# LuxGraph/Lux

Measured on NVIDIA H100. Metric: MTEPS, higher is better.
Workload: dtype f32

## Files before the change

lux_b200/csrc/api.cu:

```cuda
#include <cub/cub.cuh>
#include <stdarg.h>
#include <stdlib.h>
#include <string.h>
#include <algorithm>
#include <new>

#include "build.cuh"
#include "cf.cuh"
#include "pull.cuh"
#include "panel.cuh"
#include "seg.cuh"
#include "push.cuh"
#include "runtime.cuh"
#include <thrust/iterator/counting_iterator.h>

using namespace luxb;

enum class AppRun : uint8_t { kIterations, kConvergence, kEntry };
static constexpr char kBcRun[] = "luxb_bc_run";

struct AppInfo {
  const char* name;
  AppRun run;
  const char* entry;
  bool weights;
  bool dist_labels;
  uint32_t vbytes;
  bool check;
  bool settable;
};
static constexpr AppInfo kApps[] = {
    {"pagerank",                        AppRun::kIterations,  nullptr,          false,  false, 4,        false, true},
    {"connected components",            AppRun::kConvergence, nullptr,          false,  false, 4,        true,  true},
    {"SSSP",                            AppRun::kConvergence, nullptr,          false,  false, 4,        true,  true},
    {"col_filter",                      AppRun::kIterations,  nullptr,          true,   false, 4 * kCfK, false, true},
    {"weighted SSSP",                   AppRun::kConvergence, nullptr,          true,   true,  4,        true,  true},
    {"betweenness centrality",          AppRun::kEntry,       kBcRun,           false,  false, 8,        false, true},
    {"weighted betweenness centrality", AppRun::kEntry,       kBcRun,           true,   true,  8,        false, true},
    {"triangle counting",               AppRun::kEntry,       "luxb_tc_run",    false,  false, 8,        false, false},
    {"k-core decomposition",            AppRun::kEntry,       "luxb_kcore_run", false,  false, 4,        true,  true},
    {"k-truss decomposition",           AppRun::kEntry,       "luxb_truss_run", false,  false, 4,        true,  false},
};
static constexpr int kNumApps = sizeof(kApps) / sizeof(kApps[0]);
static_assert(kNumApps == LUXB_TRUSS + 1, "one row per luxb_app");
static const AppInfo& app_of(const luxb_graph* g) { return kApps[g->cfg.app]; }

static const char* const kPhaseName[12] = {"pull_tile", "fixup", "refresh", "rechunk", "barrier", "panel", "combine", "pack+push", "pull/bcast", "cold_hub", "bc_sigma", "bc_delta"};
static void pt_mark(luxb_graph* g, int tag) {
  PhaseTimer& pt = g->pt;
  if (!pt.on) return;
  cudaEvent_t e;
  cudaEventCreate(&e);
  cudaEventRecord(e, g->stream);
  pt.ev.push_back(e);
  pt.tag.push_back(tag);
}
static void pt_print(luxb_graph* g) {
  if (g->pt.on && g->pt.cnt) {
    char line[1024];
    const bool bc = app_of(g).entry == kBcRun;
    int n = snprintf(line, sizeof(line), "[luxb rank %d] phase means over %ld %s:", g->cfg.rank, g->pt.cnt, bc ? "sources" : "iterations");
    double sum = 0;
    for (int k = bc ? 10 : 0; k < (bc ? 12 : 10); ++k) {
      n += snprintf(line + n, sizeof(line) - n, " %s %.3f ms;", kPhaseName[k], g->pt.sum[k] / g->pt.cnt);
      sum += g->pt.sum[k] / g->pt.cnt;
    }
    snprintf(line + n, sizeof(line) - n, " sum %.3f ms\n", sum);
    fputs(line, stderr);
  }
}

static void pt_flush(luxb_graph* g) {
  PhaseTimer& pt = g->pt;
  if (!pt.on || pt.ev.empty()) return;
  cudaStreamSynchronize(g->stream);
  for (size_t i = 1; i < pt.ev.size(); ++i) {
    if (pt.tag[i] < 0) continue;
    float ms = 0;
    cudaEventElapsedTime(&ms, pt.ev[i - 1], pt.ev[i]);
    pt.sum[pt.tag[i]] += ms;
    if (pt.tag[i] == (app_of(g).entry == kBcRun ? 10 : 0)) pt.cnt++;
  }
  for (cudaEvent_t e : pt.ev) cudaEventDestroy(e);
  pt.ev.clear();
  pt.tag.clear();
}


namespace luxb {
static thread_local char g_err[1024] = "";
void set_error(const char* fmt, ...) {
  va_list ap;
  va_start(ap, fmt);
  vsnprintf(g_err, sizeof(g_err), fmt, ap);
  va_end(ap);
}
}

#define LUXB_ARG(cond, ...)             \
  do {                                  \
    if (!(cond)) {                      \
      set_error(__VA_ARGS__);           \
      return LUXB_ERR_ARG;              \
    }                                   \
  } while (0)

#define LUXB_NCCL(expr)                                                                              \
  do {                                                                                               \
    ncclResult_t _r = (expr);                                                                        \
    if (_r != ncclSuccess) {                                                                         \
      set_error("NCCL error %s at %s:%d: %s", #expr, __FILE__, __LINE__, nccl().GetErrorString(_r)); \
      return LUXB_ERR_COMM;                                                                          \
    }                                                                                                \
  } while (0)

#define LUXB_PULL_SHAPES(X) X(0, 7, 8, 2) X(1, 9, 8, 2) X(2, 7, 16, 2)
#define LUXB_DECL_SHAPE(id, ipt, warps, stages) using PullShape##id = PullShape<ipt, warps, stages>;
LUXB_PULL_SHAPES(LUXB_DECL_SHAPE)
#define LUXB_TILE_OF(id, ipt, warps, stages) PullShape##id::kTile,
static const int kPullTileOf[] = {LUXB_PULL_SHAPES(LUXB_TILE_OF)};
static const int kNumPullShapes = sizeof(kPullTileOf) / sizeof(int);
static const int kDefaultPullShape = 0;
static const int kDefaultPullCtas = 3;

static inline int grid_for(uint64_t n, int threads, int cap) {
  uint64_t b = (n + threads - 1) / threads;
  if (b < 1) b = 1;
  if (b > (uint64_t)cap) b = cap;
  return (int)b;
}

template <class T>
static size_t padded_bytes(uint64_t count) { return std::max<uint64_t>(count, 1) * sizeof(T) + 256; }

template <class T>
static int gmalloc(luxb_graph* g, T** p, uint64_t count, MemKind kind = MemKind::kDevice) {
  void* q = nullptr;
  if (kind == MemKind::kDevice) LUXB_CUDA(cudaMalloc(&q, padded_bytes<T>(count)));
  else if (kind == MemKind::kPinned) LUXB_CUDA(cudaMallocHost(&q, padded_bytes<T>(count)));
  else LUXB_CUDA(cudaHostAlloc(&q, padded_bytes<T>(count), cudaHostAllocMapped | cudaHostAllocPortable));
  g->owned.push_back({q, kind});
  *p = reinterpret_cast<T*>(q);
  return 0;
}

static cudaError_t free_owned(const OwnedBuf& b) { return b.kind == MemKind::kDevice ? cudaFree(b.p) : cudaFreeHost(b.p); }

static int gfree(luxb_graph* g, void* p) {
  for (size_t i = 0; i < g->owned.size(); ++i)
    if (g->owned[i].p == p) {
      const OwnedBuf b = g->owned[i];
      g->owned.erase(g->owned.begin() + i);
      LUXB_CUDA(free_owned(b));
      return 0;
    }
  return 0;
}

template <class T>
static int edge_alloc(luxb_graph* g, T** p, uint64_t count) {
  return gmalloc(g, p, count, g->cfg.zero_copy_edges ? MemKind::kMapped : MemKind::kDevice);
}

struct DevTmp {
  std::vector<void*> ptrs;
  ~DevTmp() { for (void* q : ptrs) cudaFree(q); }
  template <class T>
  int alloc(T** out, uint64_t count) {
    void* q = nullptr;
    LUXB_CUDA(cudaMalloc(&q, padded_bytes<T>(count)));
    ptrs.push_back(q);
    *out = reinterpret_cast<T*>(q);
    return 0;
  }
  void release(void* q) {
    for (size_t i = 0; i < ptrs.size(); ++i)
      if (ptrs[i] == q) { cudaFree(q); ptrs.erase(ptrs.begin() + i); return; }
  }
  void keep(luxb_graph* g, void* q) {
    for (size_t i = 0; i < ptrs.size(); ++i)
      if (ptrs[i] == q) { ptrs.erase(ptrs.begin() + i); g->owned.push_back({q, MemKind::kDevice}); return; }
  }
};

template <class F>
static int cub_call(DevTmp& tmp, cudaStream_t stream, F&& f) {
  size_t bytes = 0;
  LUXB_CUDA(f(nullptr, bytes));
  char* d_tmp = nullptr;
  LUXB_TRY(tmp.alloc(&d_tmp, bytes));
  LUXB_CUDA(f(d_tmp, bytes));
  LUXB_CUDA(cudaStreamSynchronize(stream));
  tmp.release(d_tmp);
  return 0;
}

static int alloc_fixup(luxb_graph* g, FixupScratch& f, uint32_t n_tiles) {
  LUXB_TRY(gmalloc(g, (uint32_t**)&f.d_head, (uint64_t)n_tiles + 1));
  LUXB_TRY(gmalloc(g, (uint32_t**)&f.d_tail, (uint64_t)n_tiles + 1));
  f.n_fix_blocks = (n_tiles + kFixBlock - 1) / kFixBlock;
  LUXB_TRY(gmalloc(g, (uint64_t**)&f.d_carry, (uint64_t)n_tiles + 1));
  LUXB_TRY(gmalloc(g, &f.d_carry_flag, (uint64_t)n_tiles + 1));
  LUXB_TRY(gmalloc(g, (uint64_t**)&f.d_block_agg, (uint64_t)f.n_fix_blocks + 1));
  LUXB_TRY(gmalloc(g, &f.d_block_flag, (uint64_t)f.n_fix_blocks + 1));
  return 0;
}

static int host_partition(uint32_t nv, uint64_t ne, const uint64_t* row_end, int P, uint32_t* rl, uint32_t* np,
                          uint64_t* cl) {
  uint64_t cap = (ne + P - 1) / P;
  uint32_t left = 0;
  int count = 0, found_adjust = 0;
  while (left < nv && count < P) {
    uint64_t base = left == 0 ? 0 : row_end[left - 1];
    const uint64_t* first = std::upper_bound(row_end + left, row_end + nv, base + cap);
    uint32_t v = (uint32_t)(first - row_end);
    if (v < nv) {
      rl[count] = left; np[count] = v - left + 1; cl[count] = base; ++count;
      left = v + 1;
    } else {
      if (row_end[nv - 1] - base == 0) --found_adjust;
      rl[count] = left; np[count] = nv - left; cl[count] = base; ++count;
      left = nv;
    }
  }
  int found = count + found_adjust;
  for (int p = count; p < P; ++p) { rl[p] = nv; np[p] = 0; cl[p] = ne; }
  return found;
}

static constexpr uint32_t kBalanceHubIndeg = 64;
static inline uint64_t vertex_cost(uint64_t indeg) { return 8 + (indeg >= kBalanceHubIndeg ? 4 : 7) * indeg; }

static void host_balanced_partition(uint32_t nv, uint64_t ne, const uint64_t* row_end, int P, uint32_t* rl, uint32_t* np, uint64_t* cl) {
  uint64_t total = 0;
  for (uint32_t v = 0; v < nv; ++v) total += vertex_cost(row_end[v] - (v ? row_end[v - 1] : 0));
  uint64_t run = 0;
  uint32_t left = 0;
  int p = 0;
  for (uint32_t v = 0; v < nv && p < P - 1; ++v) {
    run += vertex_cost(row_end[v] - (v ? row_end[v - 1] : 0));
    if (run * P >= total * (uint64_t)(p + 1)) {
      rl[p] = left; np[p] = v - left + 1; cl[p] = left ? row_end[left - 1] : 0;
      left = v + 1;
      ++p;
    }
  }
  rl[p] = left; np[p] = nv - left; cl[p] = left ? row_end[left - 1] : 0;
  for (++p; p < P; ++p) { rl[p] = nv; np[p] = 0; cl[p] = ne; }
}

static bool use_balanced_split(const luxb_config* cfg) {
  return cfg->balanced_split && cfg->nranks > 1 && (cfg->app == LUXB_PAGERANK || cfg->app == LUXB_COLFILTER);
}

static int check_config(const luxb_config* cfg) {
  LUXB_ARG(cfg != nullptr, "config is NULL");
  LUXB_ARG((unsigned)cfg->app < (unsigned)kNumApps, "unknown app %d", (int)cfg->app);
  LUXB_ARG(cfg->nranks >= 1 && cfg->nranks <= LUXB_MAX_PARTS, "nranks %d out of range [1,%d]", cfg->nranks, LUXB_MAX_PARTS);
  LUXB_ARG(cfg->rank >= 0 && cfg->rank < cfg->nranks, "rank %d out of range", cfg->rank);
  return 0;
}

static int graph_begin(const luxb_config* cfg, uint32_t nv, uint64_t ne, luxb_graph** out) {
  LUXB_TRY(check_config(cfg));
  LUXB_ARG(out != nullptr, "out is NULL");
  int ndev = 0;
  cudaError_t e = cudaGetDeviceCount(&ndev);
  if (e != cudaSuccess || ndev == 0) {
    set_error("no CUDA device available (%s): libluxb has no CPU fallback", cudaGetErrorString(e));
    return LUXB_ERR_CUDA;
  }
  LUXB_ARG(cfg->device >= 0 && cfg->device < ndev, "device %d out of range (have %d)", cfg->device, ndev);
  LUXB_CUDA(cudaSetDevice(cfg->device));
  luxb_graph* g = new (std::nothrow) luxb_graph();
  if (!g) { set_error("out of host memory"); return LUXB_ERR_NOMEM; }
  g->cfg = *cfg;
  g->P = cfg->nranks;
  g->nv = nv;
  g->ne = ne;
  g->weighted = app_of(g).weights;
  *out = g;
  LUXB_CUDA(cudaStreamCreateWithFlags(&g->stream, cudaStreamNonBlocking));
  LUXB_CUDA(cudaEventCreate(&g->ev_begin));
  LUXB_CUDA(cudaEventCreate(&g->ev_end));
  LUXB_CUDA(cudaDeviceGetAttribute(&g->num_sms, cudaDevAttrMultiProcessorCount, cfg->device));
  g->pull_ctas = kDefaultPullCtas;
  if (const char* env = getenv("LUXB_PULL_CTAS")) g->pull_ctas = std::max(1, atoi(env));
  if (const char* env = getenv("LUXB_PHASE_TIMING")) { g->pt.on = atoi(env) != 0; g->pt.per_call = atoi(env) == 2; }
  if (const char* env = getenv("LUXB_L2_HINTS")) g->l2_hints = atoi(env);
  if (const char* env = getenv("LUXB_OVERLAP")) g->overlap_exchange = atoi(env) != 0;
  if (const char* env = getenv("LUXB_BARRIER")) { g->flag_barrier = strcmp(env, "nccl") != 0; g->flag_barrier_all = strcmp(env, "flag") == 0; }
  if (const char* env = getenv("LUXB_PUSH")) g->direct_push = strcmp(env, "direct") == 0;
  if (const char* env = getenv("LUXB_BARRIER_TIMEOUT_S")) g->barrier_timeout_ns = (uint64_t)std::max(1, atoi(env)) * 1000000000ull;
  if (const char* env = getenv("LUXB_FUSED_FIXUP")) g->fused_fixup = atoi(env) != 0;
  if (const char* env = getenv("LUXB_PANEL_RESERVE_SMS")) g->panel_reserve_sms = std::max(0, atoi(env));
  return 0;
}

static void set_partition_derived(luxb_graph* g) {
  int r = g->cfg.rank;
  g->row_left = g->rl[r];
  g->n_part = g->np[r];
  g->col_left = g->cl[r];
  uint64_t next = (r + 1 < g->P) ? g->cl[r + 1] : g->ne;
  if (g->np[r] == 0) next = g->col_left;
  g->e_part = next - g->col_left;
// ... 655 lines not shown
  std::vector<unsigned long long> hist(cap + 1);
  LUXB_CUDA(cudaMemcpyAsync(hist.data(), d_hist, (cap + 1) * 8, cudaMemcpyDeviceToHost, g->stream));
  LUXB_CUDA(cudaStreamSynchronize(g->stream));
  uint64_t above = 0;
  uint32_t tau = cap + 1;
  for (uint32_t d = cap; d >= 2; --d) {
    if (above + hist[d] > h_max) break;
    above += hist[d];
    tau = d;
  }
  if (above == 0 || tau > cap) return 0;
  const uint32_t H = (uint32_t)above;
  if (compact_cold && g->P == 1) {
    const int cs_mode = g->sweep.cs;
    uint64_t e_cold_src = 0;
    for (uint32_t d = 1; d < tau; ++d) e_cold_src += (uint64_t)d * hist[d];
    if (cs_mode == 0 || (cs_mode < 0 && (!split_may_run(g) || g->e_part < kSplitMinEdges ||
                                         (double)e_cold_src < kColdSplitMinShare * (double)g->e_part)))
      compact_cold = false;
  }
  uint64_t *d_keys = nullptr, *d_keys2 = nullptr;
  uint32_t *d_ids = nullptr, *d_ids2 = nullptr, *d_map = nullptr;
  unsigned int* d_cursor = nullptr;
  LUXB_TRY(tmp.alloc(&d_keys, H));
  LUXB_TRY(tmp.alloc(&d_keys2, H));
  LUXB_TRY(tmp.alloc(&d_ids, H));
  LUXB_TRY(tmp.alloc(&d_ids2, H));
  LUXB_TRY(gmalloc(g, &g->d_hot_order, H));
  LUXB_TRY(tmp.alloc(&d_cursor, 1 + LUXB_MAX_PARTS));
  LUXB_CUDA(cudaMemsetAsync(d_cursor, 0, 4 * (1 + LUXB_MAX_PARTS), g->stream));
  PartTable pt{};
  pt.P = g->P;
  for (int p = 0; p < g->P; ++p) { pt.rl[p] = g->rl[p]; pt.np[p] = g->np[p]; }
  hot_select_kernel<<<grid, 256, 0, g->stream>>>(g->d_deg, g->nv, tau, pt, d_cursor, d_cursor + 1, d_keys, d_ids, H);
  LUXB_CUDA(cudaGetLastError());
  int vbits = 1;
  while ((1ull << vbits) < (uint64_t)g->nv) ++vbits;
  LUXB_TRY(cub_call(tmp, g->stream, [&](void* t, size_t& b) {
    return cub::DeviceRadixSort::SortPairs(t, b, d_ids, d_ids2, d_keys, d_keys2, (int)H, 0, vbits, g->stream);
  }));
  LUXB_TRY(cub_call(tmp, g->stream, [&](void* t, size_t& b) {
    return cub::DeviceRadixSort::SortPairs(t, b, d_keys2, d_keys, d_ids2, g->d_hot_order, (int)H, 0, 32, g->stream);
  }));
  unsigned int h_cnt[1 + LUXB_MAX_PARTS];
  LUXB_CUDA(cudaMemcpyAsync(h_cnt, d_cursor, sizeof(h_cnt), cudaMemcpyDeviceToHost, g->stream));
  LUXB_CUDA(cudaStreamSynchronize(g->stream));
  g->hot_off[0] = 0;
  for (int p = 0; p < g->P; ++p) g->hot_off[p + 1] = g->hot_off[p] + h_cnt[1 + p];
  LUXB_TRY(tmp.alloc(&d_map, g->nv));
  uint32_t *d_cflag = nullptr, *d_crank = nullptr;
  if (compact_cold) {
    LUXB_TRY(tmp.alloc(&d_cflag, (uint64_t)g->nv + 1));
    LUXB_TRY(tmp.alloc(&d_crank, (uint64_t)g->nv + 1));
    cold_flag_kernel<<<grid, 256, 0, g->stream>>>(g->d_deg, g->nv, tau, d_cflag);
    LUXB_CUDA(cudaMemsetAsync(d_cflag + g->nv, 0, 4, g->stream));
    LUXB_TRY(cub_call(tmp, g->stream, [&](void* t, size_t& b) {
      return cub::DeviceScan::ExclusiveSum(t, b, d_cflag, d_crank, (int)g->nv + 1, g->stream);
    }));
    for (int p = 0; p <= g->P; ++p) {
      const uint32_t at = p < g->P ? std::min(g->rl[p], g->nv) : g->nv;
      LUXB_CUDA(cudaMemcpyAsync(&g->cold_off[p], d_crank + at, 4, cudaMemcpyDeviceToHost, g->stream));
    }
    LUXB_CUDA(cudaStreamSynchronize(g->stream));
    g->cold_n = g->cold_off[g->P];
    gather_map_compact_kernel<<<grid, 256, 0, g->stream>>>(d_map, d_crank, g->nv, H);
  } else {
    gather_map_init_kernel<<<grid, 256, 0, g->stream>>>(d_map, g->nv, H);
  }
  if (compact_cold && g->P == 1) {
    uint32_t* d_zsrc = nullptr;
    LUXB_TRY(gmalloc(g, &d_zsrc, (uint64_t)H + g->cold_n + 1));
    LUXB_CUDA(cudaMemcpyAsync(d_zsrc, g->d_hot_order, (size_t)H * 4, cudaMemcpyDeviceToDevice, g->stream));
    pack_list_cold_kernel<<<grid, 256, 0, g->stream>>>(d_cflag, d_crank, 0, g->nv, 0, d_zsrc + H);
    LUXB_CUDA(cudaGetLastError());
    LUXB_CUDA(cudaStreamSynchronize(g->stream));
    LUXB_TRY(gfree(g, g->d_hot_order));
    g->d_hot_order = d_zsrc;
    g->cold_z = true;
  } else if (compact_cold) {
    uint32_t *d_okeys = nullptr, *d_okeys2 = nullptr, *d_ranks = nullptr;
    LUXB_TRY(tmp.alloc(&d_okeys, H));
    LUXB_TRY(tmp.alloc(&d_okeys2, H));
    LUXB_TRY(tmp.alloc(&d_ranks, H));
    LUXB_TRY(gmalloc(g, &g->d_zperm, H));
    owner_keys_kernel<<<grid, 256, 0, g->stream>>>(g->d_hot_order, H, pt, d_okeys, d_ranks);
    LUXB_CUDA(cudaGetLastError());
    LUXB_TRY(cub_call(tmp, g->stream, [&](void* t, size_t& b) {
      return cub::DeviceRadixSort::SortPairs(t, b, d_okeys, d_okeys2, d_ranks, g->d_zperm, (int)H, 0, 8, g->stream);
    }));
    const int me = g->cfg.rank;
    const uint32_t nh_me = g->hot_off[me + 1] - g->hot_off[me], nc_me = g->cold_off[me + 1] - g->cold_off[me];
    LUXB_TRY(gmalloc(g, &g->d_pack_list, (uint64_t)nh_me + nc_me + 1));
    if (nh_me)
      pack_list_hot_kernel<<<grid_for(nh_me, 256, grid), 256, 0, g->stream>>>(g->d_hot_order, g->d_zperm, g->hot_off[me], nh_me, g->row_left,
                                                                              g->d_pack_list);
    if (g->n_part)
      pack_list_cold_kernel<<<grid, 256, 0, g->stream>>>(d_cflag, d_crank, g->row_left, g->n_part, g->cold_off[me], g->d_pack_list + nh_me);
    LUXB_CUDA(cudaGetLastError());
    g->packed = true;
  }
  gather_map_hot_kernel<<<grid, 256, 0, g->stream>>>(d_map, g->d_hot_order, H);
  LUXB_TRY(edge_alloc(g, &g->d_src_gather, g->e_part + 8));
  LUXB_CUDA(cudaMemsetAsync(g->d_src_gather, 0, (g->e_part + 8) * 4, g->stream));
  remap_src_kernel<<<grid, 256, 0, g->stream>>>(g->d_src, g->e_part, d_map, g->d_src_gather);
  LUXB_CUDA(cudaGetLastError());
  LUXB_CUDA(cudaStreamSynchronize(g->stream));
  g->hot_n = H;
  return 0;
}

static int allgather_slices(luxb_graph* g, void* replica, size_t elem_bytes);
static void resolve_sweep_settings(SweepSettings& s);
static int build_seg_sweep(luxb_graph* g);
static int pagerank_publish(luxb_graph* g, float* x_new);
static int wait_cold_exchange(luxb_graph* g);
static int bc_alloc(luxb_graph* g);
static int tc_build(luxb_graph* g);
static int kcore_build(luxb_graph* g);
static int truss_build(luxb_graph* g);

static int build_gather_side(luxb_graph* g, bool compact_cold, bool streams) {
  LUXB_TRY(gmalloc(g, &g->d_deg, g->nv));
  LUXB_CUDA(cudaMemsetAsync(g->d_deg, 0, (size_t)g->nv * 4, g->stream));
  hist_src_kernel<<<g->num_sms * 8, 256, 0, g->stream>>>(g->d_src, g->e_part, g->d_deg);
  LUXB_CUDA(cudaGetLastError());
  if (g->P > 1) LUXB_NCCL(nccl().AllReduce(g->d_deg, g->d_deg, g->nv, ncclUint32, ncclSum, g->comm, g->stream));
  LUXB_TRY(build_hot_layout(g, compact_cold));
  if (streams) LUXB_TRY(build_seg_sweep(g));
  if (g->hot_n) {
    const uint64_t z_len = (uint64_t)g->hot_n + (g->cold_z ? g->cold_n : 0) + 65536;
    LUXB_TRY(gmalloc(g, (uint32_t**)&g->d_hot, z_len));
    LUXB_CUDA(cudaMemsetAsync(g->d_hot, 0, z_len * 4, g->stream));
    LUXB_TRY(set_l2_persisting_window(g, g->d_hot, (size_t)g->hot_n * 4));
  }
  return 0;
}

int luxb_init(luxb_graph* g) {
  LUXB_ARG(g != nullptr, "graph is NULL");
  if (g->inited) { set_error("luxb_init called twice"); return LUXB_ERR_STATE; }
  if (g->P > 1 && !g->comm) { set_error("luxb_init: nranks > 1 needs luxb_comm_init first"); return LUXB_ERR_STATE; }
  LUXB_CUDA(cudaSetDevice(g->cfg.device));
  resolve_sweep_settings(g->sweep);
  const int grid = g->num_sms * 8;
  switch (g->cfg.app) {
    case LUXB_PAGERANK: {
      LUXB_TRY(build_gather_side(g, true, true));
      for (int k = 0; k < 2; ++k) LUXB_TRY(gmalloc(g, (float**)&g->d_val[k], (uint64_t)g->nv + 64));
      pr_init_kernel<<<grid, 256, 0, g->stream>>>(g->d_deg, g->nv, (float*)g->d_val[0]);
      LUXB_CUDA(cudaMemsetAsync(g->d_val[1], 0, (size_t)g->nv * 4, g->stream));
      if (g->packed) {
        g->xt_hot_chunk = ((((uint64_t)g->hot_n + g->P - 1) / g->P) + 31) & ~31ull;
        g->xt_cold_chunk = ((((uint64_t)g->cold_n + g->P - 1) / g->P) + 31) & ~31ull;
        const uint64_t xt_len = (g->xt_hot_chunk + g->xt_cold_chunk) * g->P;
        for (int k = 0; k < 2; ++k) {
          LUXB_TRY(gmalloc(g, &g->d_xt[k], xt_len));
          LUXB_CUDA(cudaMemsetAsync(g->d_xt[k], 0, xt_len * 4, g->stream));
        }
      }
      LUXB_CUDA(cudaGetLastError());
      LUXB_TRY(pagerank_publish(g, (float*)g->d_val[0]));
      g->replica_stale = false;
      break;
    }
    case LUXB_COLFILTER: {
      for (int k = 0; k < 2; ++k) LUXB_TRY(gmalloc(g, (float**)&g->d_val[k], (uint64_t)g->nv * kCfK));
      cf_init_kernel<<<grid, 256, 0, g->stream>>>((float*)g->d_val[0], (uint64_t)g->nv * kCfK);
      cf_init_kernel<<<grid, 256, 0, g->stream>>>((float*)g->d_val[1], (uint64_t)g->nv * kCfK);
      DevTmp tmp;
      uint32_t* d_cnt = nullptr;
      LUXB_TRY(tmp.alloc(&d_cnt, (uint64_t)g->n_part + 1));
      LUXB_TRY(gmalloc(g, &g->cf.chunk_first, (uint64_t)g->n_part + 2));
      LUXB_CUDA(cudaMemsetAsync(d_cnt, 0, ((size_t)g->n_part + 1) * 4, g->stream));
      cf_chunk_count_kernel<<<grid, 256, 0, g->stream>>>(g->d_row_end, g->n_part, d_cnt);
      LUXB_TRY(cub_call(tmp, g->stream, [&](void* t, size_t& b) {
        return cub::DeviceScan::ExclusiveSum(t, b, d_cnt, g->cf.chunk_first, (int)g->n_part + 1, g->stream);
      }));
      LUXB_CUDA(cudaMemcpyAsync(&g->cf.n_chunks, g->cf.chunk_first + g->n_part, 4, cudaMemcpyDeviceToHost, g->stream));
      LUXB_CUDA(cudaStreamSynchronize(g->stream));
      tmp.release(d_cnt);
      LUXB_TRY(gmalloc(g, &g->cf.chunk_vtx, g->cf.n_chunks));
      LUXB_TRY(gmalloc(g, &g->cf.partial, (uint64_t)g->cf.n_chunks * kCfK));
      cf_chunk_fill_kernel<<<grid, 256, 0, g->stream>>>(g->cf.chunk_first, g->n_part, g->cf.chunk_vtx);
      LUXB_CUDA(cudaGetLastError());
      break;
    }
    case LUXB_CC:
    case LUXB_SSSP:
    case LUXB_SSSP_WEIGHTED:
    case LUXB_BC:
    case LUXB_BC_WEIGHTED: {
      LUXB_ARG(app_of(g).run != AppRun::kConvergence || g->cfg.app == LUXB_CC || g->cfg.start_vtx < g->nv, "start vertex %u >= nv",
               g->cfg.start_vtx);
      LUXB_TRY(gmalloc(g, (uint32_t**)&g->d_val[0], g->nv));
      LUXB_TRY(gmalloc(g, &g->d_cur, g->n_part));
      LUXB_TRY(build_push_csr(g));
      LUXB_TRY(build_gather_side(g, false, !app_of(g).dist_labels));
      g->big_capacity = (uint32_t)std::min<uint64_t>(g->e_part / kPushBigDegree + 1024, 0x7FFFFFFFull);
      LUXB_TRY(gmalloc(g, (PushArgs::BigSeg**)&g->d_big_list, g->big_capacity));
      LUXB_TRY(gmalloc(g, &g->d_fq_all, g->fq_total));
      LUXB_TRY(gmalloc(g, &g->d_fq_new, g->slot_bytes[g->cfg.rank]));
      LUXB_TRY(gmalloc(g, &g->d_fq_tmp, g->slot_bytes[g->cfg.rank]));
      LUXB_TRY(gmalloc(g, &g->d_hdr_all, 2 * LUXB_MAX_PARTS));
      LUXB_TRY(gmalloc(g, &g->h_hdr, 2 * LUXB_MAX_PARTS, MemKind::kPinned));
      LUXB_TRY(gmalloc(g, &g->h_scratch, 16, MemKind::kPinned));
      LUXB_TRY(reset_label_state(g, false, g->cfg.start_vtx));
      if (g->P > 1) {
        LUXB_NCCL(nccl().AllGather(g->d_fq_new, g->d_hdr_all, 8, ncclUint8, g->comm, g->stream));
        LUXB_TRY(allgather_slices(g, g->d_val[0], 4));
        LUXB_CUDA(cudaStreamSynchronize(g->stream));
      }
      if (app_of(g).entry == kBcRun) LUXB_TRY(bc_alloc(g));
      break;
    }
    case LUXB_TC: LUXB_TRY(tc_build(g)); break;
    case LUXB_KCORE: LUXB_TRY(kcore_build(g)); break;
    case LUXB_TRUSS: LUXB_TRY(truss_build(g)); break;
  }
  LUXB_CUDA(cudaStreamSynchronize(g->stream));
  g->cur = 0;
  g->inited = true;
  return 0;
}

static int allgather_slices(luxb_graph* g, void* replica, size_t elem_bytes) {
  if (g->P == 1) return 0;
  LUXB_NCCL(nccl().GroupStart());
  for (int p = 0; p < g->P; ++p) {
    if (g->np[p] == 0) continue;
    char* ptr = reinterpret_cast<char*>(replica) + (size_t)g->rl[p] * elem_bytes;
    LUXB_NCCL(nccl().Broadcast(ptr, ptr, (size_t)g->np[p] * elem_bytes, ncclUint8, p, g->comm, g->stream));
  }
  LUXB_NCCL(nccl().GroupEnd());
  return 0;
}

static int p2p_barrier(luxb_graph* g) {
  if (g->P == 1) return 0;
  if (g->flag_barrier && g->p2p_ready && (g->cfg.app == LUXB_PAGERANK || g->flag_barrier_all)) {
    FlagBarrierArgs a{};
    for (int p = 0; p < g->P; ++p) a.peer[p] = reinterpret_cast<uint32_t*>(g->peer_flags[p]);
    a.mine = g->d_flags;
    a.err = g->h_barrier_err;
    a.P = g->P;
    a.me = g->cfg.rank;
    a.epoch = ++g->barrier_epoch;
    a.timeout_ns = g->barrier_timeout_ns;
    flag_barrier_kernel<<<1, LUXB_MAX_PARTS, 0, g->stream>>>(a);
    LUXB_CUDA(cudaGetLastError());
    g->stats.kernel_launches++;
    return 0;
  }
  if (!g->d_sync) LUXB_TRY(gmalloc(g, &g->d_sync, 4));
  LUXB_NCCL(nccl().AllReduce(g->d_sync, g->d_sync, 1, ncclUint32, ncclSum, g->comm, g->stream));
  return 0;
}

extern "C++" {
template <class Prog, class Shape>
static int launch_pull_shape(luxb_graph* g, const PullArgs<Prog>& a) {
  auto kern = pull_tile_kernel<Prog, Shape>;
  const int want = g->pull_ctas;
  constexpr size_t smem = pull_smem_bytes<Prog, Shape>();
  LUXB_CUDA(cudaFuncSetAttribute(kern, cudaFuncAttributeMaxDynamicSharedMemorySize, (int)smem));
  int carve_pct = (int)std::min<size_t>(100, (want * (smem + 1024) * 100 + 228 * 1024 - 1) / (228 * 1024));
  LUXB_CUDA(cudaFuncSetAttribute(kern, cudaFuncAttributePreferredSharedMemoryCarveout, carve_pct));
  const uint32_t n_super = (a.n_tiles + Shape::kWarps - 1) / Shape::kWarps;
  uint32_t grid = (uint32_t)std::min<uint64_t>((uint64_t)g->num_sms * want, n_super);
  kern<<<grid, Shape::kThreads, smem, g->stream>>>(a);
  LUXB_CUDA(cudaGetLastError());
  return 0;
}

static int kt_begin(luxb_graph* g) {
  if (!g->kernel_timing) return 0;
  if (g->kt_used + 2 > g->kt_events.size()) {
    cudaEvent_t e0, e1;
    LUXB_CUDA(cudaEventCreate(&e0));
    LUXB_CUDA(cudaEventCreate(&e1));
    g->kt_events.push_back(e0);
    g->kt_events.push_back(e1);
  }
  LUXB_CUDA(cudaEventRecord(g->kt_events[g->kt_used], g->stream));
  return 0;
}
static int kt_end(luxb_graph* g) {
  if (!g->kernel_timing) return 0;
  LUXB_CUDA(cudaEventRecord(g->kt_events[g->kt_used + 1], g->stream));
  g->kt_used += 2;
  return 0;
}

template <class Prog>
static void fill_fixup_args(PullArgs<Prog>& a, const FixupScratch& f) {
  a.head_partial = reinterpret_cast<typename Prog::Acc*>(f.d_head);
  a.tail_partial = reinterpret_cast<typename Prog::Acc*>(f.d_tail);
  a.carry = reinterpret_cast<typename Prog::Wide*>(f.d_carry);
  a.carry_flag = f.d_carry_flag;
  a.block_agg = reinterpret_cast<typename Prog::Wide*>(f.d_block_agg);
  a.block_flag = f.d_block_flag;
}

template <class Prog>
static int launch_fixup(luxb_graph* g, const PullArgs<Prog>& a, FixupScratch& f) {
  if (a.n_tiles <= 1) return 0;
  if (g->fused_fixup) {
    if (!f.d_chain) {
      LUXB_TRY(gmalloc(g, &f.d_chain, 4ull * f.n_fix_blocks + 4));
      LUXB_CUDA(cudaMemsetAsync(f.d_chain, 0, (4ull * f.n_fix_blocks + 4) * 8, g->stream));
      f.chain_epoch = 0;
    }
    FixupChain<Prog> ch;
    ch.value = f.d_chain;
    ch.status = f.d_chain + 2ull * f.n_fix_blocks;
    ch.ticket = f.d_chain + 4ull * f.n_fix_blocks;
    ch.n_blocks = f.n_fix_blocks;
    ch.epoch = ++f.chain_epoch;
    if (f.chain_epoch >= 0x3FFFFFF0u) {
      LUXB_CUDA(cudaMemsetAsync(f.d_chain, 0, (4ull * f.n_fix_blocks + 4) * 8, g->stream));
      f.chain_epoch = ch.epoch = 1;
    }
    pull_fixup_fused_kernel<Prog><<<f.n_fix_blocks, kFixBlock, 0, g->stream>>>(a, ch);
    LUXB_CUDA(cudaGetLastError());
    g->stats.kernel_launches++;
    return 0;
  }
  pull_fixup_scan_kernel<Prog><<<f.n_fix_blocks, kFixBlock, 0, g->stream>>>(a);
  pull_fixup_blocks_kernel<Prog><<<1, 1024, 0, g->stream>>>(a, f.n_fix_blocks);
  pull_fixup_apply_kernel<Prog><<<f.n_fix_blocks, kFixBlock, 0, g->stream>>>(a);
  LUXB_CUDA(cudaGetLastError());
  g->stats.kernel_launches += 3;
  return 0;
}

template <class Prog>
static int launch_pull(luxb_graph* g, PullLayout& L, const uint32_t* src, const typename Prog::Vertex* x_nat,
                       const typename Prog::Vertex* x_cold, const typename Prog::Vertex* x_hot, uint32_t hot_n,
                       typename Prog::Vertex* out_local, const typename Prog::Params& prm, const uint32_t* hub_bits = nullptr,
                       bool timed = true) {
  if (L.n_tiles == 0) return 0;
  PullArgs<Prog> a{};
  a.row_end = L.d_row_end;
  a.row_end32 = L.d_row_end32;
  a.src = src;
  a.x_nat = x_nat;
  a.n_part = L.n_vtx;
  a.e_part = L.e_cnt;
  a.row_left = g->row_left;
  a.x_old = x_cold;
  a.x_hot = x_hot;
  a.hot_n = hot_n;
  a.out = out_local;
  a.tile_v = L.d_tile_v;
  a.n_tiles = L.n_tiles;
  fill_fixup_args(a, L.fix);
  a.tile_counter = reinterpret_cast<uint32_t*>(g->d_counters + 2);
  LUXB_CUDA(cudaMemsetAsync(a.tile_counter, 0, 4, g->stream));
  a.prm = prm;
  a.hub_bits = hub_bits;
  a.raw_out = 0;
  if constexpr (Prog::kWeighted) a.weight = g->d_weight;
  if (timed) LUXB_TRY(kt_begin(g));
  switch (g->pull_shape) {
#define LUXB_CASE_SHAPE(id, ipt, warps, stages) \
    case id: LUXB_TRY((launch_pull_shape<Prog, PullShape##id>(g, a))); break;
    LUXB_PULL_SHAPES(LUXB_CASE_SHAPE)
    default: set_error("bad pull shape"); return LUXB_ERR_STATE;
  }
  if (timed) LUXB_TRY(kt_end(g));
  g->stats.kernel_launches++;
  pt_mark(g, 0);
  LUXB_TRY(launch_fixup(g, a, L.fix));
  pt_mark(g, 1);
  return 0;
}
}

#define LUXB_SEG_MAIN_SHAPES(X) X(0, 8, 2, 2) X(1, 8, 3, 1) X(2, 12, 2, 1) X(3, 8, 2, 4) X(4, 16, 2, 1) X(5, 8, 4, 1) X(6, 8, 2, 1) X(7, 6, 2, 2)
#define LUXB_DECL_MSHAPE(id, warps, stages, rounds) using SegMain##id = SegShape<warps, stages, rounds, false, 0>;
LUXB_SEG_MAIN_SHAPES(LUXB_DECL_MSHAPE)
#define LUXB_SEG_PANEL_SHAPES(X) \
  X(0, 31, 2, 2, 32768, 8) X(1, 24, 2, 1, 32768, 16) X(2, 16, 2, 2, 32768, 16) X(3, 24, 2, 2, 32768, 8) X(4, 20, 2, 1, 32768, 16) X(5, 16, 2, 4, 32768, 8)
#define LUXB_DECL_PSHAPE(id, warps, stages, rounds, tab, v) using SegPanel##id = SegShape<warps, stages, rounds, true, tab, v>;
LUXB_SEG_PANEL_SHAPES(LUXB_DECL_PSHAPE)
struct SegShapeInfo { int piece, stage_edges, tab; };
#define LUXB_MSHAPE_INFO(id, warps, stages, rounds) {SegMain##id::kPiece, SegMain##id::kStageEdges, 0},
#define LUXB_PSHAPE_INFO(id, warps, stages, rounds, tab, v) {SegPanel##id::kPiece, SegPanel##id::kStageEdges, SegPanel##id::kTab},
static const SegShapeInfo kSegMainInfo[] = {LUXB_SEG_MAIN_SHAPES(LUXB_MSHAPE_INFO)};
static const SegShapeInfo kSegPanelInfo[] = {LUXB_SEG_PANEL_SHAPES(LUXB_PSHAPE_INFO)};
static const int kNumSegMain = sizeof(kSegMainInfo) / sizeof(SegShapeInfo);
static const int kNumSegPanel = sizeof(kSegPanelInfo) / sizeof(SegShapeInfo);

static int env_int(const char* name, int dflt) {
  const char* e = getenv(name);
  return e ? atoi(e) : dflt;
}

static double env_double(const char* name, double dflt) {
  const char* e = getenv(name);
  return e ? atof(e) : dflt;
}

static void resolve_sweep_settings(SweepSettings& s) {
  s = SweepSettings();
  if (const char* e = getenv("LUXB_SWEEP")) s.seg = strcmp(e, "merge") != 0;
  auto shape = [](const char* name, int dflt, int n) { const int v = env_int(name, dflt); return v < 0 || v >= n ? 0 : v; };
  s.main_shape = shape("LUXB_SEG_MAIN_SHAPE", s.main_shape, kNumSegMain);
  s.panel_shape = shape("LUXB_SEG_PANEL_SHAPE", s.panel_shape, kNumSegPanel);
  s.cs_shape = shape("LUXB_CS_SHAPE", s.main_shape, kNumSegMain);
  s.sb = env_int("LUXB_SB", s.sb);
  const int tab = kSegPanelInfo[s.panel_shape].tab;
  s.sb_bs = std::min<uint32_t>((uint32_t)std::max(4, env_int("LUXB_SB_BS", tab)) & ~3u, (uint32_t)tab);
  s.sb_blocks = (uint32_t)std::min(std::max(env_int("LUXB_SB_BLOCKS", (int)s.sb_blocks), 1), kPanelMaxBlocks);
  s.sb_min_indeg = (uint32_t)std::max(env_int("LUXB_SB_MIN_INDEG", (int)s.sb_min_indeg), 1);
  s.sb_tier = env_int("LUXB_SB_TIER", s.sb_tier);
  s.sb_slot_edges = env_double("LUXB_SB_SLOT_EDGES", s.sb_slot_edges);
  s.cs = env_int("LUXB_CS", s.cs);
  s.cs_seg_mb = env_double("LUXB_CS_SEG_MB", s.cs_seg_mb);
  s.hot_mb = env_double("LUXB_HOT_MB", s.hot_mb);
  s.l2_persist = env_int("LUXB_L2_PERSIST", 1) != 0;
  s.l2_window_mb = env_double("LUXB_L2_WINDOW_MB", s.l2_window_mb);
}

extern "C++" {
template <class Word, class In>
static int build_seg_stream(luxb_graph* g, PullLayout& L, const uint64_t* d_row_end, uint32_t n_vtx, const In* d_ids, uint64_t e_cnt,
                            StreamBlocks& blk, uint32_t stage_edges, uint32_t piece, uint32_t vtx_offset, bool want_empty,
                            const uint32_t* hub_bits, uint32_t* super_end) {
  const int grid = g->num_sms * 8;
  DevTmp tmp;
  L = PullLayout();
  L.n_vtx = n_vtx;
  L.e_cnt = e_cnt;
  uint64_t words = 0, pads_total = 0;
  for (uint32_t b = 0; b < blk.n_blocks; ++b) {
    const uint64_t eb = blk.ebase[b + 1] - blk.ebase[b];
    const uint64_t pad = stage_edges - eb % stage_edges;
    blk.wbase[b] = words;
    blk.hshift[b] = pads_total;
    words += eb + pad;
    pads_total += pad;
    if (super_end) super_end[b] = (uint32_t)(words / stage_edges);
  }
  blk.wbase[blk.n_blocks] = words;
  blk.hshift[blk.n_blocks] = pads_total;
  LUXB_ARG(words / piece < 0xFFFFFFF0ull && words / stage_edges < 0xFFFFFFF0ull, "stream too large");
  L.n_words = words;
  L.n_stages = (uint32_t)(words / stage_edges);
  L.n_tiles = (uint32_t)(words / piece);
  uint32_t *d_flag = nullptr, *d_rank = nullptr;
  LUXB_TRY(tmp.alloc(&d_flag, (uint64_t)n_vtx + 1));
  LUXB_TRY(tmp.alloc(&d_rank, (uint64_t)n_vtx + 1));
  nonempty_flag_kernel<<<grid, 256, 0, g->stream>>>(d_row_end, n_vtx, d_flag);
  LUXB_CUDA(cudaMemsetAsync(d_flag + n_vtx, 0, 4, g->stream));
  LUXB_TRY(cub_call(tmp, g->stream, [&](void* t, size_t& b) {
    return cub::DeviceScan::ExclusiveSum(t, b, d_flag, d_rank, (int)n_vtx + 1, g->stream);
  }));
  uint32_t n_seg = 0;
  LUXB_CUDA(cudaMemcpyAsync(&n_seg, d_rank + n_vtx, 4, cudaMemcpyDeviceToHost, g->stream));
  LUXB_CUDA(cudaStreamSynchronize(g->stream));
  Word* d_words = nullptr;
  LUXB_TRY(gmalloc(g, &d_words, words + 64));
  L.d_src = d_words;
  if (e_cnt) stream_copy_kernel<Word, In><<<grid, 256, 0, g->stream>>>(d_ids, e_cnt, blk, d_words);
  for (uint32_t b = 0; b < blk.n_blocks; ++b) {
    const uint64_t from = blk.wbase[b] + (blk.ebase[b + 1] - blk.ebase[b]);
    stream_pad_kernel<Word><<<grid_for(blk.wbase[b + 1] - from, 256, grid), 256, 0, g->stream>>>(d_words, from, blk.wbase[b + 1]);
  }
  LUXB_CUDA(cudaGetLastError());
  const uint64_t n_heads = (uint64_t)n_seg + pads_total;
  LUXB_ARG(n_heads < 0xFFFFFFF0ull, "too many segments");
  LUXB_TRY(gmalloc(g, &L.d_close, n_heads + 2));
  LUXB_CUDA(cudaMemsetAsync(L.d_close, 0xFF, (n_heads + 2) * 4, g->stream));
  stream_heads_kernel<Word><<<grid, 256, 0, g->stream>>>(d_row_end, n_vtx, d_flag, d_rank, blk, d_words, L.d_close, vtx_offset);
  LUXB_CUDA(cudaGetLastError());
  uint32_t* d_cnt = nullptr;
  LUXB_TRY(tmp.alloc(&d_cnt, (uint64_t)L.n_tiles + 2));
  LUXB_CUDA(cudaMemsetAsync(d_cnt, 0, ((size_t)L.n_tiles + 2) * 4, g->stream));
  piece_heads_kernel<Word><<<grid, 256, 0, g->stream>>>(d_words, L.n_tiles, piece, d_cnt);
  LUXB_CUDA(cudaGetLastError());
  LUXB_TRY(gmalloc(g, &L.d_tile_v, (uint64_t)L.n_tiles + 2));
  LUXB_TRY(cub_call(tmp, g->stream, [&](void* t, size_t& b) {
    return cub::DeviceScan::ExclusiveSum(t, b, d_cnt, L.d_tile_v, (int)L.n_tiles + 1, g->stream);
  }));
  uint32_t heads_counted = 0;
  LUXB_CUDA(cudaMemcpyAsync(&heads_counted, L.d_tile_v + L.n_tiles, 4, cudaMemcpyDeviceToHost, g->stream));
  unsigned int* d_cur2 = nullptr;
  if (want_empty) {
    const uint32_t n_e = n_vtx - n_seg;
    LUXB_TRY(gmalloc(g, &L.d_empty, (uint64_t)n_e + 1));
    LUXB_TRY(gmalloc(g, &L.d_empty_hub, (uint64_t)n_e + 1));
    LUXB_TRY(tmp.alloc(&d_cur2, 2));
    LUXB_CUDA(cudaMemsetAsync(d_cur2, 0, 8, g->stream));
    empty_split_kernel<<<grid, 256, 0, g->stream>>>(d_flag, n_vtx, hub_bits, L.d_empty, L.d_empty_hub, d_cur2);
    LUXB_CUDA(cudaGetLastError());
    unsigned int h_cur2[2] = {0, 0};
    LUXB_CUDA(cudaMemcpyAsync(h_cur2, d_cur2, 8, cudaMemcpyDeviceToHost, g->stream));
    LUXB_CUDA(cudaStreamSynchronize(g->stream));
    L.n_empty = h_cur2[0];
    L.n_empty_hub = h_cur2[1];
  }
  LUXB_CUDA(cudaStreamSynchronize(g->stream));
  if ((uint64_t)heads_counted != n_heads) {
    set_error("flagged stream: %u heads counted, %llu expected", heads_counted, (unsigned long long)n_heads);
    return LUXB_ERR_STATE;
  }
  return alloc_fixup(g, L.fix, L.n_tiles);
}
}

static int build_main_stream(luxb_graph* g, const uint64_t* d_row_end, const uint32_t* d_ids, uint64_t e_cnt, const uint32_t* hub_bits) {
  const SegShapeInfo shp = kSegMainInfo[g->sweep.main_shape];
  StreamBlocks blk{};
  blk.n_blocks = 1;
  blk.vfirst[1] = g->n_part;
  blk.ebase[1] = e_cnt;
  return build_seg_stream<uint32_t, uint32_t>(g, g->sb_main, d_row_end, g->n_part, d_ids, e_cnt, blk, (uint32_t)shp.stage_edges,
                                              (uint32_t)shp.piece, 0, true, hub_bits, nullptr);
}

extern "C++" {
template <class Word>
static int build_group_stream(luxb_graph* g, PullLayout& L, const uint16_t* d_key, const uint64_t* d_pay, uint64_t e_cnt, uint32_t g0,
                              uint32_t g1, const unsigned long long* hist, uint32_t bs, const SegShapeInfo& shp, uint32_t* super_end) {
  const int grid = g->num_sms * 8;
  const uint32_t* vbase = g->sb_groups.vbase;
  const uint32_t v0 = vbase[g0], n_vtx = vbase[g1] - v0;
  DevTmp tmp;
  Word* d_ids = nullptr;
  uint32_t* d_vcount = nullptr;
  uint64_t* d_vrow = nullptr;
  LUXB_TRY(tmp.alloc(&d_ids, e_cnt + 32));
  LUXB_TRY(tmp.alloc(&d_vcount, (uint64_t)n_vtx + 1));
  LUXB_CUDA(cudaMemsetAsync(d_vcount, 0, ((size_t)n_vtx + 1) * 4, g->stream));
  group_fill_kernel<Word><<<grid, 256, 0, g->stream>>>(d_key, d_pay, e_cnt, g->d_src_gather, bs, g->sb_groups, v0, d_ids, d_vcount);
  LUXB_CUDA(cudaGetLastError());
  LUXB_TRY(tmp.alloc(&d_vrow, (uint64_t)n_vtx + 4));
  widen_u32_to_u64_kernel<<<grid, 256, 0, g->stream>>>(d_vcount, d_vrow, n_vtx);
  LUXB_TRY(cub_call(tmp, g->stream, [&](void* t, size_t& b) {
    return cub::DeviceScan::InclusiveSum(t, b, d_vrow, d_vrow, (int)n_vtx, g->stream);
  }));
  tmp.release(d_vcount);
  StreamBlocks blk{};
  blk.n_blocks = super_end ? g1 - g0 : 1;
  for (uint32_t b = 0; b < blk.n_blocks; ++b) {
    blk.vfirst[b + 1] = super_end ? vbase[g0 + b + 1] - v0 : n_vtx;
    blk.ebase[b + 1] = super_end ? blk.ebase[b] + hist[g0 + b] : e_cnt;
  }
  return build_seg_stream<Word, Word>(g, L, d_vrow, n_vtx, d_ids, e_cnt, blk, (uint32_t)shp.stage_edges, (uint32_t)shp.piece, v0, false,
                                      nullptr, super_end);
}
}

static int build_panel_layout(luxb_graph* g) {
  g->sb_on = false;
  g->cs_on = false;
  const SweepSettings& st = g->sweep;
  if (!split_may_run(g) || g->hot_n == 0 || g->e_part == 0 || g->e_part >= 0xFFFFFFFFull) return 0;
  const SegShapeInfo shp = kSegPanelInfo[st.panel_shape];
  const uint32_t bs = st.sb_bs;
  const uint32_t NB0 = (uint32_t)((std::min<uint64_t>(g->hot_n, (uint64_t)st.sb_blocks * bs) + bs - 1) / bs);
  const bool tiers = st.sb_tier > 0 || (st.sb_tier < 0 && g->cold_z && g->e_part >= kSplitMinEdges);
  const uint32_t nb_all = tiers ? (uint32_t)std::min<uint64_t>(((uint64_t)g->hot_n + bs - 1) / bs, kPanelMaxBlocks) : NB0;
  const int grid = g->num_sms * 8;
  DevTmp tmp;

  uint32_t *d_flag = nullptr, *d_hub_idx = nullptr;
  LUXB_TRY(tmp.alloc(&d_flag, (uint64_t)g->n_part + 1));
  LUXB_TRY(tmp.alloc(&d_hub_idx, (uint64_t)g->n_part + 1));
  hub_flag_kernel<<<grid, 256, 0, g->stream>>>(g->d_row_end, g->n_part, st.sb_min_indeg, d_flag);
  LUXB_CUDA(cudaGetLastError());
  LUXB_TRY(cub_call(tmp, g->stream, [&](void* t, size_t& b) {
    return cub::DeviceScan::ExclusiveSum(t, b, d_flag, d_hub_idx, (int)g->n_part, g->stream);
  }));
  uint32_t last_idx = 0, last_flag = 0;
  LUXB_CUDA(cudaMemcpyAsync(&last_idx, d_hub_idx + g->n_part - 1, 4, cudaMemcpyDeviceToHost, g->stream));
  LUXB_CUDA(cudaMemcpyAsync(&last_flag, d_flag + g->n_part - 1, 4, cudaMemcpyDeviceToHost, g->stream));
  LUXB_CUDA(cudaStreamSynchronize(g->stream));
  const uint32_t Nh = last_idx + last_flag;
  if (Nh == 0 || (uint64_t)Nh * NB0 >= 0x7FFFFFF0ull) return 0;
  uint32_t *d_hub_vtx = nullptr, *d_hub_bits = nullptr, *d_cov = nullptr;
  LUXB_TRY(tmp.alloc(&d_hub_vtx, Nh));
  LUXB_TRY(tmp.alloc(&d_hub_bits, ((uint64_t)g->n_part + 31) / 32 + 1));
  LUXB_TRY(tmp.alloc(&d_cov, Nh));
  hub_list_kernel<<<grid, 256, 0, g->stream>>>(d_flag, d_hub_idx, g->n_part, d_hub_vtx, d_hub_bits);
  LUXB_CUDA(cudaGetLastError());
  std::vector<uint32_t> hub_key(Nh);
  {
    uint32_t *d_hkey = nullptr, *d_hkey2 = nullptr, *d_hvtx2 = nullptr;
    LUXB_TRY(tmp.alloc(&d_hkey, Nh));
    LUXB_TRY(tmp.alloc(&d_hkey2, Nh));
    LUXB_TRY(tmp.alloc(&d_hvtx2, Nh));
    hub_order_key_kernel<<<grid, 256, 0, g->stream>>>(g->d_row_end, d_hub_vtx, Nh, d_hkey);
    LUXB_CUDA(cudaGetLastError());
    LUXB_TRY(cub_call(tmp, g->stream, [&](void* t, size_t& b) {
      return cub::DeviceRadixSort::SortPairs(t, b, d_hkey, d_hkey2, d_hub_vtx, d_hvtx2, (int)Nh, 0, 32, g->stream);
    }));
    LUXB_CUDA(cudaMemcpyAsync(d_hub_vtx, d_hvtx2, (size_t)Nh * 4, cudaMemcpyDeviceToDevice, g->stream));
    hub_pos_kernel<<<grid, 256, 0, g->stream>>>(d_hub_vtx, Nh, d_hub_idx);
    LUXB_CUDA(cudaGetLastError());
    LUXB_CUDA(cudaMemcpyAsync(hub_key.data(), d_hkey2, (size_t)Nh * 4, cudaMemcpyDeviceToHost, g->stream));
    LUXB_CUDA(cudaStreamSynchronize(g->stream));
    tmp.release(d_hkey);
    tmp.release(d_hkey2);
    tmp.release(d_hvtx2);
  }
  uint32_t NB = nb_all;
  std::vector<uint32_t> n_pref(NB, Nh);
  uint32_t* d_pref = nullptr;
  LUXB_TRY(tmp.alloc(&d_pref, kPanelMaxBlocks));
  LUXB_CUDA(cudaMemcpyAsync(d_pref, n_pref.data(), (size_t)NB * 4, cudaMemcpyHostToDevice, g->stream));

  ColdSplit cs{};
  cs.hot_n = g->hot_n;
  cs.key0 = NB;
  uint32_t S = 0;
  if (g->cold_z && st.cs != 0 && g->cold_n > 0) {
    const uint32_t s_max = 255 - NB0;
    uint64_t seg = std::max<uint64_t>(1, (uint64_t)(st.cs_seg_mb * 1e6 / 4.0));
    seg = std::min<uint64_t>(std::max<uint64_t>(seg, (g->cold_n + s_max - 1) / s_max), g->cold_n);
    const uint32_t n_seg = (uint32_t)((g->cold_n + seg - 1) / seg);
    if ((uint64_t)Nh * n_seg < 0x7FFFFFF0ull) { cs.seg = (uint32_t)seg; S = n_seg; }
  }

  uint16_t *d_key = nullptr, *d_key2 = nullptr;
  uint64_t *d_pay = nullptr, *d_pay2 = nullptr;
  LUXB_TRY(tmp.alloc(&d_key, g->e_part));
  LUXB_TRY(tmp.alloc(&d_key2, g->e_part));
  LUXB_TRY(tmp.alloc(&d_pay, g->e_part));
  LUXB_TRY(tmp.alloc(&d_pay2, g->e_part));
  constexpr int kBins = kSplitKeyMain + 1;
  unsigned long long* d_hist = nullptr;
  LUXB_TRY(tmp.alloc(&d_hist, kBins));
  unsigned long long hist[kBins];
  auto key_edges = [&]() -> int {
    const uint32_t n_src = (uint32_t)std::min<uint64_t>(g->hot_n, (uint64_t)NB * bs);
    edge_iota_kernel<<<grid, 256, 0, g->stream>>>(d_pay, d_key, g->e_part);
    hub_key_kernel<<<grid, 256, 0, g->stream>>>(g->d_row_end, g->d_src_gather, d_hub_vtx, Nh, n_src, bs, d_pref, NB, d_key, d_pay, d_cov, cs);
    LUXB_CUDA(cudaMemsetAsync(d_hist, 0, kBins * 8, g->stream));
    key_hist_kernel<<<grid, 256, 0, g->stream>>>(d_key, g->e_part, d_hist);
    LUXB_CUDA(cudaGetLastError());
    LUXB_CUDA(cudaMemcpyAsync(hist, d_hist, sizeof(hist), cudaMemcpyDeviceToHost, g->stream));
    LUXB_CUDA(cudaStreamSynchronize(g->stream));
    return 0;
  };
  LUXB_TRY(key_edges());
  bool rekey = false;
  if (tiers && NB > NB0) {
    uint64_t e_hub = 0;
    for (uint32_t h = 0; h < Nh; ++h) e_hub += ~hub_key[h];
    for (uint32_t b = NB0; b < NB; ++b) {
      uint32_t keep = 0;
      if (hist[b] > 0) {
        const double d_min = st.sb_slot_edges * (double)e_hub / (double)hist[b];
        keep = (uint32_t)(std::partition_point(hub_key.begin(), hub_key.end(), [&](uint32_t k) { return (double)~k >= d_min; }) - hub_key.begin());
      }
      n_pref[b] = std::min(keep, n_pref[b - 1]);
      rekey |= n_pref[b] < Nh;
    }
    while (NB > NB0 && n_pref[NB - 1] == 0) --NB;
    cs.key0 = NB;
    LUXB_CUDA(cudaMemcpyAsync(d_pref, n_pref.data(), (size_t)NB * 4, cudaMemcpyHostToDevice, g->stream));
  }
  uint64_t e_cs = 0;
  for (uint32_t s = 0; s < S; ++s) e_cs += hist[nb_all + s];
  if (S && st.cs < 0 && !(e_cs > 0 && (double)e_cs >= kColdSplitMinShare * (double)g->e_part)) {
    rekey |= e_cs > 0;
    cs.seg = 0;
    S = 0;
  }
  if (rekey) LUXB_TRY(key_edges());
  {
    cub::DoubleBuffer<uint16_t> kb(d_key, d_key2);
    cub::DoubleBuffer<uint64_t> pb(d_pay, d_pay2);
    int hbits = 1;
    while ((1ull << hbits) < (uint64_t)Nh) ++hbits;
    LUXB_TRY(cub_call(tmp, g->stream, [&](void* t, size_t& b) {
      return cub::DeviceRadixSort::SortPairs(t, b, pb, kb, (long long)g->e_part, 32, 32 + hbits, g->stream);
    }));
    LUXB_TRY(cub_call(tmp, g->stream, [&](void* t, size_t& b) {
      return cub::DeviceRadixSort::SortPairs(t, b, kb, pb, (long long)g->e_part, 0, kSplitKeyBits, g->stream);
    }));
    tmp.release(kb.Alternate());
    tmp.release(pb.Alternate());
    d_key2 = kb.Current();
    d_pay2 = pb.Current();
  }
  uint64_t e_cov = 0, e_cov0 = 0, e_cold = 0;
  for (uint32_t b = 0; b < NB; ++b) e_cov += hist[b];
  for (uint32_t b = 0; b < NB0; ++b) e_cov0 += hist[b];
  for (uint32_t s = 0; s < S; ++s) e_cold += hist[NB + s];
  const uint64_t e_main = hist[kSplitKeyMain];
  if (e_cov + e_cold + e_main != g->e_part) {
    set_error("panel split lost edges (%llu + %llu + %llu != %llu)", (unsigned long long)e_cov, (unsigned long long)e_cold,
              (unsigned long long)e_main, (unsigned long long)g->e_part);
    return LUXB_ERR_STATE;
  }
  if (e_cov == 0 || (st.sb < 0 && e_cov < g->e_part / 5)) return 0;

  const uint32_t NG = NB + S;
  LUXB_ARG(NG < kSplitKeyMain, "panel: too many source groups");
  uint64_t n_slots = 0;
  g->sb_groups = SplitGroups{};
  for (uint32_t k = 0; k < NG; ++k) {
    n_slots += k < NB ? n_pref[k] : Nh;
    LUXB_ARG(n_slots < 0x7FFFFFF0ull, "panel: too many (group, hub) slots");
    g->sb_groups.vbase[k + 1] = (uint32_t)n_slots;
  }
  LUXB_TRY(build_group_stream<uint16_t>(g, g->sb_panel, d_key2, d_pay2, e_cov, 0, NB, hist, bs, shp, g->sb_super_end));
  if (S)
    LUXB_TRY(build_group_stream<uint32_t>(g, g->sb_cold, d_key2 + e_cov, d_pay2 + e_cov, e_cold, NB, NG, hist, 0,
                                          kSegMainInfo[st.cs_shape], nullptr));

  uint32_t* d_main_src = nullptr;
  uint64_t* d_main_row = nullptr;
  LUXB_TRY(tmp.alloc(&d_main_src, e_main + 8));
  main_fill_kernel<<<grid, 256, 0, g->stream>>>(d_pay2 + e_cov + e_cold, e_main, g->d_src_gather, d_main_src);
  LUXB_TRY(tmp.alloc(&d_main_row, (uint64_t)g->n_part + 4));
  main_indeg_kernel<<<grid, 256, 0, g->stream>>>(g->d_row_end, g->n_part, d_flag, d_hub_idx, d_cov, d_main_row);
  LUXB_CUDA(cudaGetLastError());
  LUXB_TRY(cub_call(tmp, g->stream, [&](void* t, size_t& b) {
    return cub::DeviceScan::InclusiveSum(t, b, d_main_row, d_main_row, (int)g->n_part, g->stream);
  }));
  uint64_t chk = 0;
  LUXB_CUDA(cudaMemcpyAsync(&chk, d_main_row + g->n_part - 1, 8, cudaMemcpyDeviceToHost, g->stream));
  LUXB_CUDA(cudaStreamSynchronize(g->stream));
  if (chk != e_main) { set_error("panel split: offsets do not add up"); return LUXB_ERR_STATE; }
  tmp.release(d_key2);
  tmp.release(d_pay2);
  LUXB_TRY(build_main_stream(g, d_main_row, d_main_src, e_main, d_hub_bits));
  tmp.release(d_main_row);
  tmp.release(d_main_src);

  LUXB_TRY(gmalloc(g, &g->d_sb_partial, (uint64_t)n_slots + 1));
  LUXB_CUDA(cudaMemsetAsync(g->d_sb_partial, g->cfg.app == LUXB_SSSP || g->cfg.app == LUXB_BC ? 0xFF : 0, ((size_t)n_slots + 1) * 4, g->stream));
  LUXB_CUDA(cudaStreamSynchronize(g->stream));
  g->d_hub_vtx = d_hub_vtx; tmp.keep(g, d_hub_vtx);
  g->d_hub_bits = d_hub_bits; tmp.keep(g, d_hub_bits);
  g->sb_n_hub = Nh;
  g->sb_n_blocks = NB;
  g->sb_n_groups = NG;
  g->sb_bs = bs;
  g->sb_on = true;
  g->cs_on = S > 0;
  const uint64_t NV = g->sb_groups.vbase[NB];
  g->stats.panel_edges = e_cov0;
  g->stats.panel_hubs = Nh;
  g->stats.panel_blocks = NB0;
  g->stats.cold_hub_edges = e_cold;
  g->stats.cold_hub_segments = S;
  g->stats.tier_blocks = NB - NB0;
  g->stats.tier_slots = NV - (uint64_t)NB0 * Nh;
  g->stats.tier_edges = e_cov - e_cov0;
  if (g->cfg.verbose)
    printf("[luxb rank %d] source-blocked sweep: %u hub destinations (in-degree >= %u) x %u blocks of %u hot sources, + %u tier blocks "
           "(%llu slots, %llu edges); panel %llu edges (%.1f %%), cold-hub %llu edges (%u segments of %u values), main %llu edges\n",
           g->cfg.rank, Nh, st.sb_min_indeg, NB0, bs, NB - NB0, (unsigned long long)(NV - (uint64_t)NB0 * Nh), (unsigned long long)(e_cov - e_cov0),
           (unsigned long long)e_cov, 100.0 * e_cov / g->e_part, (unsigned long long)e_cold, S, cs.seg, (unsigned long long)e_main);
  return 0;
}

static int build_seg_sweep(luxb_graph* g) {
  g->seg_on = false;
  g->sb_on = false;
  if (!g->sweep.seg) return 0;
  if (g->n_part == 0 || g->cfg.zero_copy_edges || g->e_part >= 0xFFFFFFF0ull) return 0;
  LUXB_TRY(build_panel_layout(g));
  if (!g->sb_on) LUXB_TRY(build_main_stream(g, g->d_row_end, g->hot_n ? g->d_src_gather : g->d_src, g->e_part, nullptr));
  g->seg_on = true;
  return 0;
}

extern "C++" {
template <class Prog, class Shape>
static int launch_seg_shape(luxb_graph* g, const SegArgs<Prog>& a, int ctas_per_sm) {
  auto kern = seg_tile_kernel<Prog, Shape>;
  const int reserve = (Shape::kPanel && g->packed) ? g->panel_reserve_sms : 0;
  LUXB_CUDA(cudaFuncSetAttribute(kern, cudaFuncAttributeMaxDynamicSharedMemorySize, (int)Shape::kSmemBytes));
  int carve_pct = (int)std::min<size_t>(100, (ctas_per_sm * (Shape::kSmemBytes + 1024) * 100 + 228 * 1024 - 1) / (228 * 1024));
  LUXB_CUDA(cudaFuncSetAttribute(kern, cudaFuncAttributePreferredSharedMemoryCarveout, carve_pct));
  const uint32_t grid = (uint32_t)std::min<uint64_t>((uint64_t)std::max(g->num_sms - reserve, 1) * ctas_per_sm, a.n_stages);
  kern<<<grid, Shape::kThreads, Shape::kSmemBytes, g->stream>>>(a);
  LUXB_CUDA(cudaGetLastError());
  return 0;
}

template <bool kPanel, class Prog>
static int launch_seg_stream(luxb_graph* g, PullLayout& L, SegArgs<Prog>& a, int shape, int ctas_per_sm, int counter_slot, int tag,
                             const char* name) {
  a.p.tile_v = L.d_tile_v;
  a.p.n_tiles = L.n_tiles;
  fill_fixup_args(a.p, L.fix);
  a.p.close_vtx = L.d_close;
  a.words = L.d_src;
  a.n_stages = L.n_stages;
  a.tile_counter = reinterpret_cast<uint32_t*>(g->d_counters + counter_slot);
  LUXB_CUDA(cudaMemsetAsync(a.tile_counter, 0, 4, g->stream));
#define LUXB_CASE_MSHAPE(id, warps, stages, rounds) \
  case id: LUXB_TRY((launch_seg_shape<Prog, SegMain##id>(g, a, ctas_per_sm))); break;
#define LUXB_CASE_PSHAPE(id, warps, stages, rounds, tab, v) \
  case id: LUXB_TRY((launch_seg_shape<Prog, SegPanel##id>(g, a, ctas_per_sm))); break;
  if constexpr (kPanel) {
    switch (shape) {
      LUXB_SEG_PANEL_SHAPES(LUXB_CASE_PSHAPE)
      default: set_error("bad %s shape", name); return LUXB_ERR_STATE;
    }
  } else {
    switch (shape) {
      LUXB_SEG_MAIN_SHAPES(LUXB_CASE_MSHAPE)
      default: set_error("bad %s shape", name); return LUXB_ERR_STATE;
    }
  }
  g->stats.kernel_launches++;
  pt_mark(g, tag);
  return launch_fixup(g, a.p, L.fix);
}
}

extern "C++" {
template <class Prog>
static int launch_seg_main(luxb_graph* g, PullLayout& L, const typename Prog::Vertex* x_nat, const typename Prog::Vertex* x_cold,
                           typename Prog::Vertex* out_local, int out_buffer, const typename Prog::Params& prm, const uint32_t* hub_bits) {
  SegArgs<Prog> a{};
  a.p.n_part = L.n_vtx;
  a.p.row_left = g->row_left;
  a.p.x_nat = x_nat;
  a.p.x_old = x_cold;
  a.p.x_hot = reinterpret_cast<const typename Prog::Vertex*>(g->d_hot);
  a.p.hot_n = g->hot_n;
  a.p.out = out_local;
  a.p.prm = prm;
  a.p.hub_bits = hub_bits;
  a.p.l2_hints = g->l2_hints;
  LUXB_TRY(wait_cold_exchange(g));
  LUXB_TRY((launch_seg_stream<false, Prog>(g, L, a, g->sweep.main_shape, g->pull_ctas, 2, 0, "seg")));
  if (out_buffer >= 0 && L.n_empty && !g->empties_done[out_buffer]) {
    empties_kernel<Prog><<<grid_for(L.n_empty, 256, g->num_sms * 8), 256, 0, g->stream>>>(a.p, L.d_empty, L.n_empty);
    g->empties_done[out_buffer] = true;
    g->stats.kernel_launches++;
  }
  if (L.n_empty_hub) {
    empties_kernel<Prog><<<grid_for(L.n_empty_hub, 256, g->num_sms * 8), 256, 0, g->stream>>>(a.p, L.d_empty_hub, L.n_empty_hub);
    g->stats.kernel_launches++;
  }
  LUXB_CUDA(cudaGetLastError());
  pt_mark(g, 1);
  return 0;
}

template <class Prog>
static int sweep_seg(luxb_graph* g, const typename Prog::Vertex* x_nat, const typename Prog::Vertex* x_cold, typename Prog::Vertex* out_local,
                     int out_buffer, const typename Prog::Params& prm) {
  using Acc = typename Prog::Acc;
  LUXB_TRY(kt_begin(g));
  if (g->sb_on) {
    SegArgs<Prog> pa{};
    pa.p.x_hot = reinterpret_cast<const typename Prog::Vertex*>(g->d_hot);
    pa.p.out = reinterpret_cast<typename Prog::Vertex*>(g->d_sb_partial);
    pa.p.raw_out = 1;
    pa.p.prm = prm;
    pa.bs = g->sb_bs;
    pa.n_blocks = g->sb_n_blocks;
    for (uint32_t b = 0; b < g->sb_n_blocks; ++b) pa.super_end[b] = g->sb_super_end[b];
    LUXB_TRY((launch_seg_stream<true, Prog>(g, g->sb_panel, pa, g->sweep.panel_shape, 1, 4, 5, "panel")));
    pt_mark(g, 1);
  }
  if (g->cs_on) {
    SegArgs<Prog> ca{};
    ca.p.x_old = x_cold;
    ca.p.x_hot = reinterpret_cast<const typename Prog::Vertex*>(g->d_hot);
    ca.p.hot_n = g->hot_n;
    ca.p.out = reinterpret_cast<typename Prog::Vertex*>(g->d_sb_partial);
    ca.p.raw_out = 1;
    ca.p.l2_hints = 0;
    ca.p.prm = prm;
    LUXB_TRY((launch_seg_stream<false, Prog>(g, g->sb_cold, ca, g->sweep.cs_shape, g->pull_ctas, 4, 9, "cold-hub")));
    pt_mark(g, 1);
  }
  LUXB_TRY((launch_seg_main<Prog>(g, g->sb_main, x_nat, x_cold, out_local, out_buffer, prm, g->sb_on ? g->d_hub_bits : nullptr)));
  LUXB_TRY(kt_end(g));
  if (g->sb_on) {
    CombineArgs<Prog> ca{};
    ca.hub_vtx = g->d_hub_vtx;
    ca.n_hub = g->sb_n_hub;
    ca.n_blocks = g->sb_n_blocks;
    ca.n_groups = g->sb_n_groups;
    ca.row_left = g->row_left;
    ca.sg = g->sb_groups;
    ca.partial = reinterpret_cast<const Acc*>(g->d_sb_partial);
    ca.x_nat = x_nat;
    ca.out = out_local;
    ca.prm = prm;
    combine_hub_kernel<Prog><<<grid_for(g->sb_n_hub, 256, g->num_sms * 8), 256, 0, g->stream>>>(ca);
    LUXB_CUDA(cudaGetLastError());
    g->stats.kernel_launches++;
    pt_mark(g, 6);
  }
  return 0;
}
}

static int pagerank_publish(luxb_graph* g, float* x_new) {
  const int me = g->cfg.rank;
  const int grid = g->num_sms * 8;
  if (g->P == 1 || !g->packed) {
    if (g->P > 1) { LUXB_TRY(allgather_slices(g, x_new, 4)); pt_mark(g, 3); }
    if (g->hot_n) {
      const uint32_t z_n = g->hot_n + (g->cold_z ? g->cold_n : 0);
      hot_refresh_kernel<float><<<grid_for(z_n, 256, grid), 256, 0, g->stream>>>((float*)g->d_hot, x_new, g->d_hot_order, 0, z_n);
      LUXB_CUDA(cudaGetLastError());
      g->stats.kernel_launches++;
      pt_mark(g, 2);
    }
    return 0;
  }
  LUXB_TRY(wait_cold_exchange(g));
  float* XTn = g->d_xt[1 - g->cur_xt];
  const uint32_t H = g->hot_n;
  const uint64_t Ch = g->xt_hot_chunk, Cc = g->xt_cold_chunk, cold_base = Ch * g->P;
  const uint32_t nh_me = g->hot_off[me + 1] - g->hot_off[me], nc_me = g->cold_off[me + 1] - g->cold_off[me];
  const bool p2p = g->p2p_ready && g->cfg.exchange != LUXB_EXCHANGE_NCCL;
  if (p2p) {
    if (nh_me + nc_me) {
      PackPushArgs<float> pa{};
      pa.x_local = x_new + g->row_left;
      pa.list = g->d_pack_list;
      pa.n_hot = nh_me;
      pa.n_cold = nc_me;
      pa.hot_pos0 = g->hot_off[me];
      pa.cold_pos0 = g->cold_off[me];
      pa.hot_chunk = Ch;
      pa.cold_chunk = Cc;
      pa.cold_base = cold_base;
      for (int k = 0; k < g->P; ++k) pa.xt[k] = reinterpret_cast<float*>(g->peer_xt[1 - g->cur_xt][k]);
      pa.P = g->P;
      const int pgrid = grid_for((uint64_t)nh_me + nc_me, 256, grid);
      if (g->direct_push) pack_push_kernel<float, true><<<pgrid, 256, 0, g->stream>>>(pa);
      else pack_push_kernel<float, false><<<pgrid, 256, 0, g->stream>>>(pa);
      LUXB_CUDA(cudaGetLastError());
      g->stats.kernel_launches++;
    }
    pt_mark(g, 7);
    LUXB_TRY(p2p_barrier(g));
    pt_mark(g, 4);
    auto pull = [&](uint64_t base, uint64_t C, cudaStream_t st, int ctas) -> int {
      ChunkPullArgs ca{};
      ca.dst = XTn + base;
      for (int k = 0; k < g->P; ++k) ca.src[k] = reinterpret_cast<const float*>(g->peer_xt[1 - g->cur_xt][k]) + base;
      ca.chunk = C;
      ca.P = g->P;
      ca.me = me;
      chunk_pull_kernel<<<ctas, 512, 0, st>>>(ca);
      LUXB_CUDA(cudaGetLastError());
      g->stats.kernel_launches++;
      return 0;
    };
    if (g->direct_push) {
    } else if (g->overlap_exchange) {
      LUXB_CUDA(cudaEventRecord(g->ev_pack, g->stream));
      LUXB_TRY(pull(0, Ch, g->stream, g->num_sms * 2));
      LUXB_CUDA(cudaStreamWaitEvent(g->stream2, g->ev_pack, 0));
      LUXB_TRY(pull(cold_base, Cc, g->stream2, std::max(2 * g->panel_reserve_sms, 8)));
      LUXB_CUDA(cudaEventRecord(g->ev_cold, g->stream2));
      g->cold_pending = true;
    } else {
      LUXB_TRY(pull(0, Ch, g->stream, g->num_sms * 2));
      LUXB_TRY(pull(cold_base, Cc, g->stream, g->num_sms * 2));
    }
    pt_mark(g, 8);
  } else {
    if (nh_me + nc_me) {
      pack_values_kernel<float><<<grid_for((uint64_t)nh_me + nc_me, 256, grid), 256, 0, g->stream>>>(
          x_new + g->row_left, g->d_pack_list, nh_me, nc_me, XTn + g->hot_off[me], XTn + cold_base + g->cold_off[me]);
      LUXB_CUDA(cudaGetLastError());
      g->stats.kernel_launches++;
    }
    pt_mark(g, 7);
    LUXB_NCCL(nccl().GroupStart());
    for (int p = 0; p < g->P; ++p) {
      const uint32_t nh = g->hot_off[p + 1] - g->hot_off[p], nc = g->cold_off[p + 1] - g->cold_off[p];
      if (nh) LUXB_NCCL(nccl().Broadcast(XTn + g->hot_off[p], XTn + g->hot_off[p], nh, ncclFloat32, p, g->comm, g->stream));
      if (nc) LUXB_NCCL(nccl().Broadcast(XTn + cold_base + g->cold_off[p], XTn + cold_base + g->cold_off[p], nc, ncclFloat32, p, g->comm,
                                         g->stream));
    }
    LUXB_NCCL(nccl().GroupEnd());
    pt_mark(g, 8);
  }
  hot_permute_kernel<float><<<grid_for(H, 256, grid), 256, 0, g->stream>>>((float*)g->d_hot, XTn, g->d_zperm, H);
  LUXB_CUDA(cudaGetLastError());
  g->stats.kernel_launches++;
  pt_mark(g, 2);
  g->cur_xt ^= 1;
  g->replica_stale = true;
  return 0;
}

static int wait_cold_exchange(luxb_graph* g) {
  if (g->cold_pending) {
    LUXB_CUDA(cudaStreamWaitEvent(g->stream, g->ev_cold, 0));
    g->cold_pending = false;
  }
  return 0;
}

static int pagerank_iteration(luxb_graph* g) {
  pt_mark(g, -1);
  PageRankProgram::Params prm;
  prm.init_rank = (1.0f - kAlpha) / (float)g->nv;
  prm.deg = g->d_deg;
  float* x_old = (float*)g->d_val[g->cur];
  float* x_new = (float*)g->d_val[1 - g->cur];
  const float* x_cold = g->packed ? g->d_xt[g->cur_xt] + g->xt_hot_chunk * g->P : g->cold_z ? (const float*)g->d_hot + g->hot_n : x_old;
  if (g->seg_on) {
    LUXB_TRY((sweep_seg<PageRankProgram>(g, x_old, x_cold, x_new + g->row_left, 1 - g->cur, prm)));
  } else {
    LUXB_TRY(wait_cold_exchange(g));
    LUXB_TRY(launch_pull<PageRankProgram>(g, g->base, g->hot_n ? g->d_src_gather : g->d_src, x_old, x_cold, (const float*)g->d_hot,
                                          g->hot_n, x_new + g->row_left, prm));
  }
  LUXB_TRY(pagerank_publish(g, x_new));
  g->cur ^= 1;
  g->stats.edges_processed += g->e_part;
  return 0;
}

static int colfilter_iteration(luxb_graph* g) {
  float* x_old = (float*)g->d_val[g->cur];
  float* x_new = (float*)g->d_val[1 - g->cur];
  if (g->n_part) {
    CfArgs a{};
    a.row_end = g->d_row_end;
    a.src = g->d_src;
    a.weight = g->d_weight;
    a.chunk_first = g->cf.chunk_first;
    a.chunk_vtx = g->cf.chunk_vtx;
    a.n_part = g->n_part;
    a.n_chunks = g->cf.n_chunks;
    a.row_left = g->row_left;
    a.x_old = x_old;
    a.partial = g->cf.partial;
    a.out = x_new + (size_t)g->row_left * kCfK;
    a.n_peers = 0;
    if (g->p2p_ready && g->cfg.exchange != LUXB_EXCHANGE_NCCL)
      for (int p = 0; p < g->P; ++p)
        if (p != g->cfg.rank) a.peer_out[a.n_peers++] = (float*)g->peer_val[1 - g->cur][p] + (size_t)g->row_left * kCfK;
    uint64_t warps = g->cf.n_chunks;
    int grid = (int)std::min<uint64_t>((warps * 32 + 255) / 256, (uint64_t)g->num_sms * 8);
    cf_chunk_kernel<<<grid, 256, 0, g->stream>>>(a);
    cf_update_kernel<<<grid_for((uint64_t)g->n_part * kCfK, 256, g->num_sms * 8), 256, 0, g->stream>>>(a);
    LUXB_CUDA(cudaGetLastError());
    g->stats.kernel_launches += 2;
  }
  if (g->P > 1) {
    if (g->p2p_ready && g->cfg.exchange != LUXB_EXCHANGE_NCCL) LUXB_TRY(p2p_barrier(g));
    else LUXB_TRY(allgather_slices(g, x_new, 4 * kCfK));
  }
  g->cur ^= 1;
  g->stats.edges_processed += g->e_part;
  return 0;
}

extern "C++" {
template <class Prog>
static int label_iteration(luxb_graph* g) {
  const int me = g->cfg.rank;
  uint32_t* lab = reinterpret_cast<uint32_t*>(g->d_val[0]);
  uint64_t old_size = 0;
  int dense_parts = 0, sparse_parts = 0;
  for (int p = 0; p < g->P; ++p) {
    old_size += g->h_hdr[2 * p + 1];
    if (g->h_hdr[2 * p] == LUXB_DENSE_BITMAP) dense_parts++; else sparse_parts++;
  }
  bool dense_fq = dense_parts >= sparse_parts;
  const bool pull = old_size > (uint64_t)(g->nv / 16);
  if (pull) dense_fq = true;
  const uint32_t max_nodes = g->cap[me];
  unsigned char* new_slot = g->d_fq_new;
  LUXB_CUDA(cudaMemsetAsync(new_slot, 0, 8, g->stream));

  if (pull) {
    typename Prog::Params prm{0};
    if (g->hot_n) {
      hot_refresh_kernel<uint32_t><<<grid_for(g->hot_n, 256, g->num_sms * 8), 256, 0, g->stream>>>((uint32_t*)g->d_hot, lab, g->d_hot_order, 0, g->hot_n);
      g->stats.kernel_launches++;
    }
    bool swept = false;
    if constexpr (!Prog::kWeighted) {
      if (g->seg_on) {
        LUXB_TRY((sweep_seg<Prog>(g, lab, lab, g->d_cur, -1, prm)));
        swept = true;
      }
    }
    if (!swept)
      LUXB_TRY(launch_pull<Prog>(g, g->base, g->hot_n ? g->d_src_gather : g->d_src, lab, lab, (const uint32_t*)g->d_hot, g->hot_n,
                                 g->d_cur, prm));
    g->stats.edges_processed += g->e_part;
    g->stats.pull_iterations++;
  } else if (g->n_part && old_size) {
    PushArgs a{};
    uint64_t blocks = 0;
    for (int p = 0; p < g->P; ++p) {
      a.fr[p].slot = slot_ptr(g->d_fq_all, g, p);
      a.fr[p].row_left = g->rl[p];
      a.fr[p].n_part = g->np[p];
      a.fr[p].type = g->h_hdr[2 * p];
      a.fr[p].count = std::min(g->h_hdr[2 * p + 1], g->cap[p]);
      uint32_t entries = a.fr[p].type == LUXB_DENSE_BITMAP ? (g->h_hdr[2 * p + 1] ? g->np[p] : 0) : a.fr[p].count;
      if (a.fr[p].type == LUXB_DENSE_BITMAP && g->h_hdr[2 * p + 1] == 0) a.fr[p].n_part = 0;
      blocks += (entries + kPushThreads - 1) / kPushThreads;
    }
    a.n_parts = g->P;
    a.out_end = g->d_out_end;
    a.out_dst = g->d_out_dst;
    a.lab = lab;
    a.cur = g->d_cur;
    a.row_left = g->row_left;
    a.new_sparse = dense_fq ? 0 : 1;
    a.new_count = reinterpret_cast<uint32_t*>(new_slot) + 1;
    a.new_queue = reinterpret_cast<uint32_t*>(new_slot + 8);
    a.max_nodes = max_nodes;
    a.edges_scanned = g->d_counters;
    a.big_list = reinterpret_cast<PushArgs::BigSeg*>(g->d_big_list);
    a.big_count = reinterpret_cast<uint32_t*>(g->d_counters + 3);
    a.big_capacity = g->big_capacity;
    a.out_w = g->d_out_w;
    if (blocks) {
      LUXB_CUDA(cudaMemsetAsync(a.big_count, 0, 4, g->stream));
      push_relax_kernel<Prog><<<(unsigned)blocks, kPushThreads, 0, g->stream>>>(a);
      push_big_kernel<Prog><<<g->num_sms * 4, kPushThreads, 0, g->stream>>>(a);
      LUXB_CUDA(cudaGetLastError());
      g->stats.kernel_launches += 2;
    }
  }

  const int fgrid = grid_for(g->n_part, 256, g->num_sms * 8);
  uint32_t count = 0;
  uint64_t total = 0;
  FrontierHeader my_hdr{LUXB_SPARSE_QUEUE, 0};
  const bool dev_frontier = g->P == 1 || (g->p2p_ready && g->cfg.exchange != LUXB_EXCHANGE_NCCL);
  if (dev_frontier) {
    unsigned char* slot_d = dense_fq ? new_slot : g->d_fq_tmp;
    unsigned char* slot_s = dense_fq ? g->d_fq_tmp : new_slot;
    LUXB_CUDA(cudaMemsetAsync(dense_fq ? slot_s : slot_d, 0, 8, g->stream));
    if (!g->d_fctl) LUXB_TRY(gmalloc(g, &g->d_fctl, 1));
    if (dense_fq) frontier_diff_kernel<<<fgrid, 256, 0, g->stream>>>(lab + g->row_left, g->d_cur, g->n_part, slot_d);
    frontier_fix_kernel<<<1, 32, 0, g->stream>>>(slot_d, slot_s, max_nodes, dense_fq ? 1 : 0, g->d_fctl);
    frontier_d2s_if_kernel<<<fgrid, 256, 0, g->stream>>>(&g->d_fctl->need_d2s, slot_d, g->row_left, g->n_part, slot_s, max_nodes);
    frontier_diff_if_kernel<<<fgrid, 256, 0, g->stream>>>(&g->d_fctl->need_promote, lab + g->row_left, g->d_cur, g->n_part, slot_d);
    frontier_final_kernel<<<1, 32, 0, g->stream>>>(slot_d, slot_s, dense_fq ? 1 : 0, g->d_fctl);
    frontier_pack_labels_if_kernel<<<grid_for(max_nodes, 256, g->num_sms * 4), 256, 0, g->stream>>>(&g->d_fctl->final_sparse, slot_s, max_nodes,
                                                                                                  g->row_left, g->d_cur);
    LUXB_CUDA(cudaGetLastError());
    g->stats.kernel_launches += dense_fq ? 6 : 5;
    if (g->P > 1) LUXB_TRY(p2p_barrier(g));
    FrontierPushArgs fa{};
    fa.ctl = g->d_fctl;
    fa.slot_d = slot_d;
    fa.slot_s = slot_s;
    fa.cur = g->d_cur;
    fa.n_part = g->n_part;
    fa.cap = g->cap[me];
    fa.row_left = g->row_left;
    fa.n_dst = 0;
    for (int p = 0; p < g->P; ++p) {
      unsigned char* fq_p = (p == me) ? g->d_fq_all : reinterpret_cast<unsigned char*>(g->peer_fq[p]);
      uint32_t* lab_p = (p == me) ? lab : reinterpret_cast<uint32_t*>(g->peer_val[0][p]);
      fa.dst_slot[fa.n_dst] = fq_p + g->slot_off[me];
      fa.dst_lab[fa.n_dst] = lab_p;
      fa.n_dst++;
    }
    frontier_push_kernel<<<g->num_sms * 2, 512, 0, g->stream>>>(fa);
    LUXB_CUDA(cudaGetLastError());
    g->stats.kernel_launches++;
    if (g->P > 1) LUXB_TRY(p2p_barrier(g));
    PartTable pt{};
    pt.P = g->P;
    if (!g->d_slot_off) {
      LUXB_TRY(gmalloc(g, &g->d_slot_off, LUXB_MAX_PARTS));
      LUXB_CUDA(cudaMemcpyAsync(g->d_slot_off, g->slot_off, sizeof(uint64_t) * g->P, cudaMemcpyHostToDevice, g->stream));
    }
    frontier_headers_kernel<<<1, LUXB_MAX_PARTS, 0, g->stream>>>(g->d_fq_all, pt, g->d_slot_off, g->d_hdr_all);
    LUXB_CUDA(cudaMemcpyAsync(g->h_hdr, g->d_hdr_all, (size_t)g->P * 8, cudaMemcpyDeviceToHost, g->stream));
    LUXB_CUDA(cudaStreamSynchronize(g->stream));
    my_hdr.type = g->h_hdr[2 * me];
    my_hdr.num_nodes = count = g->h_hdr[2 * me + 1];
    for (int p = 0; p < g->P; ++p) total += g->h_hdr[2 * p + 1];
  } else {
    if (dense_fq) {
      if (g->n_part) {
        frontier_diff_kernel<<<fgrid, 256, 0, g->stream>>>(lab + g->row_left, g->d_cur, g->n_part, new_slot);
        g->stats.kernel_launches++;
// ... 1304 lines not shown
```

lux_b200/csrc/panel.cuh:

```cuda
#pragma once
#include "common.cuh"
#include "programs.cuh"
#include "pull.cuh"

namespace luxb {

constexpr int kPanelMaxBlocks = 256;
constexpr uint16_t kSplitKeyMain = 511;
constexpr int kSplitKeyBits = 9;

struct SplitGroups {
  uint32_t vbase[kSplitKeyMain + 1];
};

__global__ void hub_flag_kernel(const uint64_t* __restrict__ row_end_rel, uint32_t n_part, uint32_t min_indeg,
                                uint32_t* __restrict__ flag) {
  for (uint64_t i = (uint64_t)blockIdx.x * blockDim.x + threadIdx.x; i < n_part; i += (uint64_t)gridDim.x * blockDim.x) {
    uint64_t d = row_end_rel[i] - (i == 0 ? 0 : row_end_rel[i - 1]);
    flag[i] = d >= min_indeg ? 1u : 0u;
  }
}

__global__ void hub_list_kernel(const uint32_t* __restrict__ flag, const uint32_t* __restrict__ hub_idx, uint32_t n_part,
                                uint32_t* __restrict__ hub_vtx, uint32_t* __restrict__ hub_bits) {
  const uint64_t n_round = ((uint64_t)n_part + 31) & ~31ull;
  for (uint64_t v = (uint64_t)blockIdx.x * blockDim.x + threadIdx.x; v < n_round; v += (uint64_t)gridDim.x * blockDim.x) {
    const bool f = v < n_part && flag[v];
    const unsigned m = __ballot_sync(0xffffffffu, f);
    if ((threadIdx.x & 31) == 0) hub_bits[v >> 5] = m;
    if (f) hub_vtx[hub_idx[v]] = (uint32_t)v;
  }
}

__global__ void hub_order_key_kernel(const uint64_t* __restrict__ row_end_rel, const uint32_t* __restrict__ hub_vtx, uint32_t n_hub,
                                     uint32_t* __restrict__ key) {
  for (uint64_t h = (uint64_t)blockIdx.x * blockDim.x + threadIdx.x; h < n_hub; h += (uint64_t)gridDim.x * blockDim.x) {
    const uint32_t v = hub_vtx[h];
    key[h] = ~(uint32_t)(row_end_rel[v] - (v == 0 ? 0 : row_end_rel[v - 1]));
  }
}

__global__ void hub_pos_kernel(const uint32_t* __restrict__ hub_vtx, uint32_t n_hub, uint32_t* __restrict__ hub_idx) {
  for (uint64_t h = (uint64_t)blockIdx.x * blockDim.x + threadIdx.x; h < n_hub; h += (uint64_t)gridDim.x * blockDim.x)
    hub_idx[hub_vtx[h]] = (uint32_t)h;
}

__global__ void edge_iota_kernel(uint64_t* __restrict__ payload, uint16_t* __restrict__ key, uint64_t n) {
  for (uint64_t e = (uint64_t)blockIdx.x * blockDim.x + threadIdx.x; e < n; e += (uint64_t)gridDim.x * blockDim.x) {
    payload[e] = e;
    key[e] = kSplitKeyMain;
  }
}

struct ColdSplit {
  uint32_t hot_n;
  uint32_t seg;
  uint32_t key0;
};

__global__ void hub_key_kernel(const uint64_t* __restrict__ row_end_rel, const uint32_t* __restrict__ src_gather,
                               const uint32_t* __restrict__ hub_vtx, uint32_t n_hub, uint32_t n_src, uint32_t bs,
                               const uint32_t* __restrict__ n_pref, uint32_t n_blocks,
                               uint16_t* __restrict__ key, uint64_t* __restrict__ payload, uint32_t* __restrict__ cov_count,
                               const ColdSplit cs) {
  __shared__ uint32_t s_pref[kPanelMaxBlocks];
  for (uint32_t i = threadIdx.x; i < n_blocks; i += blockDim.x) s_pref[i] = n_pref[i];
  __syncthreads();
  const unsigned lane = threadIdx.x & 31;
  const uint64_t warps_total = ((uint64_t)gridDim.x * blockDim.x) >> 5;
  for (uint64_t h = ((uint64_t)blockIdx.x * blockDim.x + threadIdx.x) >> 5; h < n_hub; h += warps_total) {
    const uint32_t v = hub_vtx[h];
    const uint64_t b = v == 0 ? 0 : row_end_rel[v - 1], e = row_end_rel[v];
    uint32_t cnt = 0;
    for (uint64_t k = b + lane; k < e; k += 32) {
      const uint32_t id = src_gather[k];
      if (id < n_src) {
        if (h < s_pref[id / bs]) {
          key[k] = (uint16_t)(id / bs);
          payload[k] = (h << 32) | k;
          ++cnt;
        }
      } else if (cs.seg != 0 && id >= cs.hot_n) {
        key[k] = (uint16_t)(cs.key0 + (id - cs.hot_n) / cs.seg);
        payload[k] = (h << 32) | k;
        ++cnt;
      }
    }
#pragma unroll
    for (int off = 16; off; off >>= 1) cnt += __shfl_xor_sync(0xffffffffu, cnt, off);
    if (lane == 0) cov_count[h] = cnt;
  }
}

__global__ void key_hist_kernel(const uint16_t* __restrict__ key, uint64_t n, unsigned long long* __restrict__ hist) {
  constexpr int kBins = kSplitKeyMain + 1;
  __shared__ unsigned int s_h[kBins];
  for (int i = threadIdx.x; i < kBins; i += blockDim.x) s_h[i] = 0;
  __syncthreads();
  for (uint64_t e = (uint64_t)blockIdx.x * blockDim.x + threadIdx.x; e < n; e += (uint64_t)gridDim.x * blockDim.x)
    atomicAdd(&s_h[key[e]], 1u);
  __syncthreads();
  for (int i = threadIdx.x; i < kBins; i += blockDim.x)
    if (s_h[i]) atomicAdd(hist + i, (unsigned long long)s_h[i]);
}

template <class Word>
__global__ void group_fill_kernel(const uint16_t* __restrict__ key_sorted, const uint64_t* __restrict__ payload_sorted, uint64_t e_cnt,
                                  const uint32_t* __restrict__ src_gather, uint32_t bs, const __grid_constant__ SplitGroups sg,
                                  uint32_t v0, Word* __restrict__ ids, uint32_t* __restrict__ vcount) {
  for (uint64_t i = (uint64_t)blockIdx.x * blockDim.x + threadIdx.x; i < e_cnt; i += (uint64_t)gridDim.x * blockDim.x) {
    const uint32_t k = key_sorted[i];
    const uint64_t p = payload_sorted[i];
    const uint32_t e = (uint32_t)p, h = (uint32_t)(p >> 32);
    ids[i] = (Word)(src_gather[e] - k * bs);
    atomicAdd(vcount + (sg.vbase[k] - v0) + h, 1u);
  }
}

__global__ void main_fill_kernel(const uint64_t* __restrict__ payload_sorted, uint64_t e_main, const uint32_t* __restrict__ src_gather,
                                 uint32_t* __restrict__ main_src) {
  for (uint64_t i = (uint64_t)blockIdx.x * blockDim.x + threadIdx.x; i < e_main; i += (uint64_t)gridDim.x * blockDim.x)
    main_src[i] = src_gather[(uint32_t)payload_sorted[i]];
}

__global__ void main_indeg_kernel(const uint64_t* __restrict__ row_end_rel, uint32_t n_part, const uint32_t* __restrict__ flag,
                                  const uint32_t* __restrict__ hub_idx, const uint32_t* __restrict__ cov_count,
                                  uint64_t* __restrict__ out) {
  for (uint64_t i = (uint64_t)blockIdx.x * blockDim.x + threadIdx.x; i < n_part; i += (uint64_t)gridDim.x * blockDim.x) {
    uint64_t d = row_end_rel[i] - (i == 0 ? 0 : row_end_rel[i - 1]);
    if (flag[i]) d -= cov_count[hub_idx[i]];
    out[i] = d;
  }
}

template <class Prog>
struct CombineArgs {
  const uint32_t* hub_vtx;
  uint32_t n_hub, n_blocks, n_groups, row_left;
  SplitGroups sg;
  const typename Prog::Acc* partial;
  const typename Prog::Vertex* x_nat;
  typename Prog::Vertex* out;
  typename Prog::Params prm;
};

template <class Prog>
__global__ void combine_hub_kernel(const __grid_constant__ CombineArgs<Prog> a) {
  for (uint64_t h = (uint64_t)blockIdx.x * blockDim.x + threadIdx.x; h < a.n_hub; h += (uint64_t)gridDim.x * blockDim.x) {
    const uint32_t v = a.hub_vtx[h];
    typename Prog::Acc raw0;
    memcpy(&raw0, &a.out[v], sizeof(raw0));
    typename Prog::Wide t = Prog::widen(raw0);
    uint32_t b = 0;
    for (; b + 8 <= a.n_blocks && h < a.sg.vbase[b + 8] - a.sg.vbase[b + 7]; b += 8) {
      typename Prog::Acc p[8];
#pragma unroll
      for (int i = 0; i < 8; ++i) p[i] = a.partial[a.sg.vbase[b + i] + h];
#pragma unroll
      for (int i = 0; i < 8; ++i) t = Prog::wcombine(t, Prog::widen(p[i]));
    }
    for (; b < a.n_blocks && h < a.sg.vbase[b + 1] - a.sg.vbase[b]; ++b)
      t = Prog::wcombine(t, Prog::widen(a.partial[a.sg.vbase[b] + h]));
    for (uint32_t k = a.n_blocks; k < a.n_groups; ++k) t = Prog::wcombine(t, Prog::widen(a.partial[a.sg.vbase[k] + h]));
    const typename Prog::Vertex oldv = Prog::kNeedsOld ? a.x_nat[a.row_left + v] : typename Prog::Vertex();
    const typename Prog::Vertex nv_ = Prog::update(a.row_left + v, Prog::narrow(t), oldv, a.prm);
    a.out[v] = nv_;
  }
}

}
```

lux_b200/csrc/pull.cuh:

```cuda
#pragma once
#include "common.cuh"
#include "programs.cuh"

namespace luxb {

template <int kIPT_, int kWarps_, int kStages_>
struct PullShape {
  static constexpr int kIPT = kIPT_;
  static constexpr int kWarps = kWarps_;
  static constexpr int kThreads = 32 * (kWarps + 1);
  static constexpr int kTile = 32 * kIPT;
  static constexpr int kSuper = kTile * kWarps;
  static constexpr int kStages = kStages_;
  static constexpr int kAElems = kSuper + 8;
  static constexpr int kEElems = kSuper + 8;
  static constexpr int kSumElems = kTile + 4;
  static constexpr int kHdrElems = kWarps + 4;
  static constexpr size_t kSmemBytes = (size_t)kStages * (kAElems + kEElems) * 4 + (size_t)kWarps * kSumElems * 4 +
                                       2 * kStages * 8 + (size_t)kStages * kHdrElems * 4 + 16;
  static_assert(kIPT % 2 == 1, "kIPT must be odd: lane-contiguous smem reads are then bank-conflict free");
  static constexpr size_t kWRingOffset = (kSmemBytes + 15) & ~(size_t)15;
};

template <class Prog, class Shape>
constexpr size_t pull_smem_bytes() {
  return Prog::kWeighted ? Shape::kWRingOffset + (size_t)Shape::kStages * Shape::kEElems * 4 : Shape::kSmemBytes;
}

template <bool kWeighted>
struct PullWeights {};
template <>
struct PullWeights<true> {
  const int32_t* weight;
};

template <class Prog>
struct PullArgs : PullWeights<Prog::kWeighted> {
  const uint64_t* row_end;
  const uint32_t* row_end32;
  const uint32_t* src;
  const uint32_t* tile_v;
  uint32_t n_part;
  uint64_t e_part;
  uint32_t n_tiles;
  uint32_t row_left;
  const typename Prog::Vertex* x_old;
  const typename Prog::Vertex* x_hot;
  uint32_t hot_n;
  const typename Prog::Vertex* x_nat;
  typename Prog::Vertex* out;
  typename Prog::Acc* head_partial;
  typename Prog::Acc* tail_partial;
  typename Prog::Wide* carry;
  uint32_t* carry_flag;
  typename Prog::Wide* block_agg;
  uint32_t* block_flag;
  uint32_t* tile_counter;
  typename Prog::Params prm;
  const uint32_t* hub_bits;
  int raw_out;
  int l2_hints;
  const uint32_t* close_vtx;
};

template <class Prog>
__device__ __forceinline__ bool store_raw(const PullArgs<Prog>& a, uint32_t v) {
  if (a.raw_out) return true;
  return a.hub_bits != nullptr && ((__ldg(a.hub_bits + (v >> 5)) >> (v & 31)) & 1u);
}

template <class Prog>
__device__ __forceinline__ void store_vertex(const PullArgs<Prog>& a, uint32_t v, typename Prog::Acc sum) {
  using Vertex = typename Prog::Vertex;
  if (store_raw(a, v)) {
    Vertex r;
    static_assert(sizeof(Vertex) == sizeof(typename Prog::Acc), "raw sums travel in the value slot");
    memcpy(&r, &sum, sizeof(r));
    a.out[v] = r;
    return;
  }
  Vertex oldv = Prog::kNeedsOld ? __ldg(a.x_nat + a.row_left + v) : Vertex();
  Vertex nv_ = Prog::update(a.row_left + v, sum, oldv, a.prm);
  a.out[v] = nv_;
}

__global__ void tile_table_kernel(const uint64_t* __restrict__ row_end, uint32_t n_part, uint64_t e_part, uint32_t tile,
                                  uint32_t n_tiles, uint32_t* __restrict__ tile_v) {
  uint32_t t = blockIdx.x * blockDim.x + threadIdx.x;
  if (t > n_tiles) return;
  uint64_t total = (uint64_t)n_part + e_part;
  uint64_t d = (uint64_t)t * tile;
  if (d > total) d = total;
  uint64_t lo = d > e_part ? d - e_part : 0, hi = d < n_part ? d : n_part;
  while (lo < hi) {
    uint64_t mid = (lo + hi) >> 1;
    if (row_end[mid] <= d - 1 - mid) lo = mid + 1; else hi = mid;
  }
  tile_v[t] = (uint32_t)lo;
}

#ifndef LUXB_GATHER_HINTS
#define LUXB_GATHER_HINTS 1
#endif
template <class T>
__device__ __forceinline__ T gather_load(const T* p, bool hot) {
#if LUXB_GATHER_HINTS
  uint32_t v;
  if (hot) asm volatile("ld.global.nc.L1::evict_last.b32 %0, [%1];" : "=r"(v) : "l"(p));
  else asm volatile("ld.global.nc.L1::no_allocate.b32 %0, [%1];" : "=r"(v) : "l"(p));
  T r;
  memcpy(&r, &v, 4);
  return r;
#else
  (void)hot;
  return __ldg(p);
#endif
}

template <class T>
__device__ __forceinline__ T gather_load_l2(const T* p, bool hot, uint64_t pol_hot, uint64_t pol_cold) {
  uint32_t v;
  if (hot) asm volatile("ld.global.nc.L1::evict_last.L2::cache_hint.b32 %0, [%1], %2;" : "=r"(v) : "l"(p), "l"(pol_hot));
  else asm volatile("ld.global.nc.L1::no_allocate.L2::cache_hint.b32 %0, [%1], %2;" : "=r"(v) : "l"(p), "l"(pol_cold));
  T r;
  memcpy(&r, &v, 4);
  return r;
}
__device__ __forceinline__ uint64_t l2_policy_evict_normal() {
  uint64_t pol;
  asm volatile("createpolicy.fractional.L2::evict_normal.b64 %0, 1.0;" : "=l"(pol));
  return pol;
}

__device__ __forceinline__ void mbar_arrive(uint64_t* bar) {
  asm volatile("mbarrier.arrive.shared::cta.b64 _, [%0];" ::"r"(smem_u32(bar)) : "memory");
}

template <class Prog, class Shape>
__global__ void __launch_bounds__(Shape::kThreads) pull_tile_kernel(const __grid_constant__ PullArgs<Prog> a) {
  using Acc = typename Prog::Acc;
  using Vertex = typename Prog::Vertex;
  static_assert(sizeof(Acc) == 4 && sizeof(Vertex) == 4, "4-byte vertex values");
  constexpr int kIPT = Shape::kIPT, kTile = Shape::kTile, kStages = Shape::kStages, kWarps = Shape::kWarps;

  extern __shared__ __align__(128) unsigned char smem_raw[];
  uint32_t* a_buf = reinterpret_cast<uint32_t*>(smem_raw);
  uint32_t* e_buf = a_buf + (size_t)kStages * Shape::kAElems;
  Acc* sums_all = reinterpret_cast<Acc*>(e_buf + (size_t)kStages * Shape::kEElems);
  uint64_t* full = reinterpret_cast<uint64_t*>(sums_all + (size_t)kWarps * Shape::kSumElems);
  uint64_t* empty = full + kStages;
  uint32_t* hdr_all = reinterpret_cast<uint32_t*>(empty + kStages);

  const int lane = threadIdx.x & 31, warp = threadIdx.x >> 5;
  const uint64_t total = (uint64_t)a.n_part + a.e_part;
  const uint32_t n_super = (a.n_tiles + kWarps - 1) / kWarps;

  if (threadIdx.x == 0) {
    for (int s = 0; s < kStages; ++s) { mbar_init(&full[s], 1); mbar_init(&empty[s], kWarps); }
    fence_mbar_init();
  }
  __syncthreads();

  if (warp == kWarps) {
    const uint64_t policy = l2_policy_evict_first();
    for (uint32_t n = 0;; ++n) {
      const int s = n % kStages;
      if (n >= (uint32_t)kStages) mbar_wait(&empty[s], ((n / kStages) - 1) & 1u);
      uint32_t T = 0;
      if (lane == 0) T = atomicAdd(a.tile_counter, 1u);
      T = __shfl_sync(0xffffffffu, T, 0);
      uint32_t* hdr = hdr_all + s * Shape::kHdrElems;
      if (T >= n_super) {
        if (lane == 0) { hdr[0] = 0xFFFFFFFFu; mbar_arrive(&full[s]); }
        break;
      }
      const uint64_t t0 = (uint64_t)T * kWarps;
      if (lane <= kWarps) {
        uint64_t tt = t0 + lane < a.n_tiles ? t0 + lane : a.n_tiles;
        hdr[1 + lane] = __ldg(a.tile_v + tt);
      }
      __syncwarp();
      if (lane == 0) {
        hdr[0] = T;
        const uint64_t t1 = t0 + kWarps < a.n_tiles ? t0 + kWarps : a.n_tiles;
        const uint32_t i0 = hdr[1], i1 = hdr[1 + kWarps];
        const uint64_t d0 = t0 * kTile, d1 = t1 * kTile < total ? t1 * kTile : total;
        const uint64_t j0 = d0 - i0, j1 = d1 - i1;
        const uint32_t is = i0 & ~3u;
        const uint32_t bytes_a = ((i1 - is + 1) * 4 + 15) & ~15u;
        const uint64_t js = j0 & ~3ull;
        uint32_t bytes_e = (uint32_t)(((j1 - js) * 4 + 15) & ~15ull);
        if (j1 == j0) bytes_e = 0;
        if constexpr (Prog::kWeighted) {
          mbar_arrive_expect_tx(&full[s], bytes_a + 2 * bytes_e);
          bulk_g2s(a_buf + (size_t)s * Shape::kAElems, a.row_end32 + is, bytes_a, &full[s], policy);
          if (bytes_e) {
            bulk_g2s(e_buf + (size_t)s * Shape::kEElems, a.src + js, bytes_e, &full[s], policy);
            int32_t* w_buf = reinterpret_cast<int32_t*>(smem_raw + Shape::kWRingOffset);
            bulk_g2s(w_buf + (size_t)s * Shape::kEElems, a.weight + js, bytes_e, &full[s], policy);
          }
        } else {
          mbar_arrive_expect_tx(&full[s], bytes_a + bytes_e);
          bulk_g2s(a_buf + (size_t)s * Shape::kAElems, a.row_end32 + is, bytes_a, &full[s], policy);
          if (bytes_e) bulk_g2s(e_buf + (size_t)s * Shape::kEElems, a.src + js, bytes_e, &full[s], policy);
        }
      }
      __syncwarp();
    }
    return;
  }

  Acc* sums = sums_all + (size_t)warp * Shape::kSumElems;
  for (uint32_t n = 0;; ++n) {
    const int s = n % kStages;
    mbar_wait(&full[s], (n / kStages) & 1u);
    const uint32_t* hdr = hdr_all + s * Shape::kHdrElems;
    const uint32_t T = hdr[0];
    if (T == 0xFFFFFFFFu) break;
    const uint64_t t0 = (uint64_t)T * kWarps;
    const uint64_t t64 = t0 + warp;
    const bool active = t64 < a.n_tiles;
    const uint32_t t = (uint32_t)t64;
    const uint32_t si0 = hdr[1];
    const uint32_t i0 = hdr[1 + warp], i1 = hdr[2 + warp];
    const uint64_t sj0 = t0 * kTile - si0;
    const uint64_t d0 = (uint64_t)t * kTile, d1 = d0 + kTile < total ? d0 + kTile : total;
    const uint64_t j0 = d0 - i0, j1 = d1 - i1;
    const uint32_t n_v = i1 - i0, n_e = active ? (uint32_t)(j1 - j0) : 0u, n_items = n_v + n_e, j0lo = (uint32_t)j0;
    const uint32_t* A = a_buf + (size_t)s * Shape::kAElems + (si0 & 3u) + (i0 - si0);
    const uint32_t* E = e_buf + (size_t)s * Shape::kEElems + (uint32_t)(sj0 & 3ull) + (uint32_t)(j0 - sj0);

    if (active) {
      uint32_t d = lane * kIPT;
      if (d > n_items) d = n_items;
      uint32_t lo = d > n_e ? d - n_e : 0, hi = d < n_v ? d : n_v;
      while (lo < hi) {
        uint32_t mid = (lo + hi) >> 1;
        if (A[mid] - j0lo <= d - 1 - mid) lo = mid + 1; else hi = mid;
      }
      uint32_t i = lo;
      const uint32_t j = d - lo;
      uint32_t i_next = __shfl_down_sync(0xffffffffu, i, 1);
      uint32_t j_next = __shfl_down_sync(0xffffffffu, j, 1);
      if (lane == 31) { i_next = n_v; j_next = n_e; }
      const uint32_t ne_lane = j_next - j;

      Acc val[kIPT];
#pragma unroll
      for (int k = 0; k < kIPT; ++k)
        if (k < (int)ne_lane) {
          const uint32_t id = E[j + k];
          const bool hot = id < a.hot_n;
          const Vertex* p = hot ? a.x_hot + id : a.x_old + (id - a.hot_n);
          if constexpr (Prog::kWeighted) {
            const int32_t* W = reinterpret_cast<const int32_t*>(smem_raw + Shape::kWRingOffset) + (size_t)s * Shape::kEElems +
                               (uint32_t)(sj0 & 3ull) + (uint32_t)(j0 - sj0);
            val[k] = Prog::gather(gather_load(p, hot), W[j + k]);
          } else {
            val[k] = Prog::gather(gather_load(p, hot));
          }
        }

      Acc acc = Prog::identity();
      bool has_c = false;
      uint32_t first_i = 0;
      Acc first_val = Prog::identity();
      uint32_t aend = A[i] - j0lo;
#pragma unroll
      for (int k = 0; k < kIPT; ++k) {
        if (k < (int)ne_lane) {
          while (i < i_next && aend <= j + k) {
            if (!has_c) { has_c = true; first_i = i; first_val = acc; } else { sums[i] = acc; }
            acc = Prog::identity();
            ++i;
            aend = A[i] - j0lo;
          }
          acc = Prog::combine(acc, val[k]);
        }
      }
      while (i < i_next) {
        if (!has_c) { has_c = true; first_i = i; first_val = acc; } else { sums[i] = acc; }
        acc = Prog::identity();
        ++i;
      }
      Acc sv = acc;
      uint32_t sf = has_c ? 1u : 0u;
#pragma unroll
      for (int off = 1; off < 32; off <<= 1) {
        Acc pv = __shfl_up_sync(0xffffffffu, sv, off);
        uint32_t pf = __shfl_up_sync(0xffffffffu, sf, off);
        if (lane >= off) {
          if (!sf) sv = Prog::combine(pv, sv);
          sf |= pf;
        }
      }
      Acc ex_v = __shfl_up_sync(0xffffffffu, sv, 1);
      if (lane == 0) ex_v = Prog::identity();
      if (has_c) sums[first_i] = Prog::combine(ex_v, first_val);
      const Acc tail = __shfl_sync(0xffffffffu, sv, 31);
      __syncwarp();
      if (lane == 0) {
        mbar_arrive(&empty[s]);
        a.tail_partial[t] = tail;
        if (n_v > 0) a.head_partial[t] = sums[0];
      }
      for (uint32_t li = lane; li < n_v; li += 32) {
        if (li == 0 && t != 0) continue;
        store_vertex<Prog>(a, i0 + li, sums[li]);
      }
      __syncwarp();
    } else {
      if (lane == 0) mbar_arrive(&empty[s]);
    }
  }
}

constexpr int kFixBlock = 256;

template <class Prog>
__device__ __forceinline__ void seg_combine(uint32_t& f2, typename Prog::Wide& v2, uint32_t f1, typename Prog::Wide v1) {
  if (!f2) v2 = Prog::wcombine(v1, v2);
  f2 |= f1;
}

template <class Prog>
__global__ void __launch_bounds__(kFixBlock) pull_fixup_scan_kernel(const __grid_constant__ PullArgs<Prog> a) {
  using Wide = typename Prog::Wide;
  __shared__ Wide s_v[kFixBlock / 32];
  __shared__ uint32_t s_f[kFixBlock / 32];
  const uint32_t t = blockIdx.x * kFixBlock + threadIdx.x;
  const int lane = threadIdx.x & 31, warp = threadIdx.x >> 5;
  uint32_t f = 0;
  Wide v = Prog::widen(Prog::identity());
  if (t < a.n_tiles) {
    f = a.tile_v[t + 1] > a.tile_v[t] ? 1u : 0u;
    v = Prog::widen(a.tail_partial[t]);
  }
  Wide sv = v;
  uint32_t sf = f;
#pragma unroll
  for (int off = 1; off < 32; off <<= 1) {
    Wide pv = __shfl_up_sync(0xffffffffu, sv, off);
    uint32_t pf = __shfl_up_sync(0xffffffffu, sf, off);
    if (lane >= off) seg_combine<Prog>(sf, sv, pf, pv);
  }
  if (lane == 31) { s_v[warp] = sv; s_f[warp] = sf; }
  __syncthreads();
  Wide wv = Prog::widen(Prog::identity());
  uint32_t wf = 0;
  for (int w = 0; w < warp; ++w) {
    uint32_t f2 = s_f[w];
    Wide v2 = s_v[w];
    seg_combine<Prog>(f2, v2, wf, wv);
    wf = f2; wv = v2;
  }
  Wide ev = __shfl_up_sync(0xffffffffu, sv, 1);
  uint32_t ef = __shfl_up_sync(0xffffffffu, sf, 1);
  if (lane == 0) { ev = Prog::widen(Prog::identity()); ef = 0; }
  seg_combine<Prog>(ef, ev, wf, wv);
  if (t < a.n_tiles) { a.carry[t] = ev; a.carry_flag[t] = ef; }
  if (threadIdx.x == kFixBlock - 1) {
    uint32_t bf = sf;
    Wide bv = sv;
    seg_combine<Prog>(bf, bv, wf, wv);
    a.block_agg[blockIdx.x] = bv;
    a.block_flag[blockIdx.x] = bf;
  }
}

template <class Prog>
__global__ void __launch_bounds__(1024) pull_fixup_blocks_kernel(const __grid_constant__ PullArgs<Prog> a, uint32_t n_blocks) {
  using Wide = typename Prog::Wide;
  __shared__ Wide s_v[32];
  __shared__ uint32_t s_f[32];
  const int lane = threadIdx.x & 31, warp = threadIdx.x >> 5;
  const uint32_t per = (n_blocks + 1023) / 1024;
  const uint32_t b0 = threadIdx.x * per < n_blocks ? threadIdx.x * per : n_blocks;
  const uint32_t b1 = b0 + per < n_blocks ? b0 + per : n_blocks;
  Wide cv = Prog::widen(Prog::identity());
  uint32_t cf = 0;
  for (uint32_t b = b0; b < b1; ++b) {
    uint32_t f2 = a.block_flag[b];
    Wide v2 = a.block_agg[b];
    seg_combine<Prog>(f2, v2, cf, cv);
    cf = f2; cv = v2;
  }
  Wide sv = cv;
  uint32_t sf = cf;
#pragma unroll
  for (int off = 1; off < 32; off <<= 1) {
    Wide pv = __shfl_up_sync(0xffffffffu, sv, off);
    uint32_t pf = __shfl_up_sync(0xffffffffu, sf, off);
    if (lane >= off) seg_combine<Prog>(sf, sv, pf, pv);
  }
  if (lane == 31) { s_v[warp] = sv; s_f[warp] = sf; }
  __syncthreads();
  Wide wv = Prog::widen(Prog::identity());
  uint32_t wf = 0;
  for (int w = 0; w < warp; ++w) {
    uint32_t f2 = s_f[w];
    Wide v2 = s_v[w];
    seg_combine<Prog>(f2, v2, wf, wv);
    wf = f2; wv = v2;
  }
  Wide pv = __shfl_up_sync(0xffffffffu, sv, 1);
  uint32_t pf = __shfl_up_sync(0xffffffffu, sf, 1);
  if (lane == 0) { pv = Prog::widen(Prog::identity()); pf = 0; }
  seg_combine<Prog>(pf, pv, wf, wv);
  for (uint32_t b = b0; b < b1; ++b) {
    uint32_t f2 = a.block_flag[b];
    Wide v2 = a.block_agg[b];
    a.block_agg[b] = pv;
    a.block_flag[b] = pf;
    seg_combine<Prog>(f2, v2, pf, pv);
    pf = f2; pv = v2;
  }
}

template <class Prog>
__global__ void __launch_bounds__(kFixBlock) pull_fixup_apply_kernel(const __grid_constant__ PullArgs<Prog> a) {
  using Wide = typename Prog::Wide;
  const uint32_t t = blockIdx.x * kFixBlock + threadIdx.x;
  if (t == 0 || t >= a.n_tiles) return;
  const uint32_t i0 = a.tile_v[t], i1 = a.tile_v[t + 1];
  if (i1 == i0) return;
  Wide c = a.carry[t];
  if (!a.carry_flag[t]) c = Prog::wcombine(a.block_agg[blockIdx.x], c);
  Wide totalw = Prog::wcombine(c, Prog::widen(a.head_partial[t]));
  uint32_t v = i0;
  if (a.close_vtx) {
    v = a.close_vtx[i0];
    if (v == 0xFFFFFFFFu) return;
  }
  store_vertex<Prog>(a, v, Prog::narrow(totalw));
}

template <class Prog>
struct FixupChain {
  unsigned long long* value;
  unsigned long long* status;
  unsigned long long* ticket;
  uint32_t epoch, n_blocks;
};

template <class Wide>
__device__ __forceinline__ unsigned long long wide_bits(Wide w) {
  unsigned long long u = 0;
  memcpy(&u, &w, sizeof(Wide));
  return u;
}
template <class Wide>
__device__ __forceinline__ Wide bits_wide(unsigned long long u) {
  Wide w;
  memcpy(&w, &u, sizeof(Wide));
  return w;
}

template <class Prog>
__global__ void __launch_bounds__(kFixBlock) pull_fixup_fused_kernel(const __grid_constant__ PullArgs<Prog> a, const FixupChain<Prog> ch) {
  using Wide = typename Prog::Wide;
  __shared__ Wide s_v[kFixBlock / 32];
  __shared__ uint32_t s_f[kFixBlock / 32];
  __shared__ Wide s_pv;
  __shared__ uint32_t s_pf;
  __shared__ uint32_t s_b;
  if (threadIdx.x == 0) s_b = (uint32_t)(atomicAdd(ch.ticket, 1ull) - (unsigned long long)(ch.epoch - 1) * ch.n_blocks);
  __syncthreads();
  const uint32_t b = s_b;
  const uint32_t t = b * kFixBlock + threadIdx.x;
  const int lane = threadIdx.x & 31, warp = threadIdx.x >> 5;
  uint32_t f = 0;
  Wide v = Prog::widen(Prog::identity());
  uint32_t i0 = 0;
  if (t < a.n_tiles) {
    i0 = a.tile_v[t];
    f = a.tile_v[t + 1] > i0 ? 1u : 0u;
    v = Prog::widen(a.tail_partial[t]);
  }
  Wide sv = v;
  uint32_t sf = f;
#pragma unroll
  for (int off = 1; off < 32; off <<= 1) {
    Wide pv = __shfl_up_sync(0xffffffffu, sv, off);
    uint32_t pf = __shfl_up_sync(0xffffffffu, sf, off);
    if (lane >= off) seg_combine<Prog>(sf, sv, pf, pv);
  }
  if (lane == 31) { s_v[warp] = sv; s_f[warp] = sf; }
  __syncthreads();
  Wide wv = Prog::widen(Prog::identity());
  uint32_t wf = 0;
  for (int w = 0; w < warp; ++w) {
    uint32_t f2 = s_f[w];
    Wide v2 = s_v[w];
    seg_combine<Prog>(f2, v2, wf, wv);
    wf = f2; wv = v2;
  }
  Wide ev = __shfl_up_sync(0xffffffffu, sv, 1);
  uint32_t ef = __shfl_up_sync(0xffffffffu, sf, 1);
  if (lane == 0) { ev = Prog::widen(Prog::identity()); ef = 0; }
  seg_combine<Prog>(ef, ev, wf, wv);
  if (threadIdx.x == kFixBlock - 1) {
    uint32_t af = sf;
    Wide av = sv;
    seg_combine<Prog>(af, av, wf, wv);
    const unsigned long long tag = (unsigned long long)ch.epoch << 2;
    volatile unsigned long long* st = ch.status;
    volatile unsigned long long* va = ch.value;
    va[2 * b] = wide_bits<Wide>(av);
    __threadfence();
    st[2 * b] = tag | (af << 1) | 1ull;
    uint32_t pf = 0;
    Wide pv = Prog::widen(Prog::identity());
    for (int64_t q = (int64_t)b - 1; q >= 0 && !pf; --q) {
      unsigned long long s_pre, s_agg;
      do {
        s_pre = st[2 * q + 1];
        s_agg = st[2 * q];
      } while ((s_pre >> 2) != ch.epoch && (s_agg >> 2) != ch.epoch);
      __threadfence();
      const bool have_prefix = (s_pre >> 2) == ch.epoch;
      uint32_t qf = (uint32_t)(((have_prefix ? s_pre : s_agg) >> 1) & 1ull);
      Wide qv = bits_wide<Wide>(va[2 * q + (have_prefix ? 1 : 0)]);
      uint32_t nf = pf;
      Wide nv_ = pv;
      seg_combine<Prog>(nf, nv_, qf, qv);
      pf = nf; pv = nv_;
      if (have_prefix) break;
    }
    uint32_t inf = af;
    Wide inv = av;
    seg_combine<Prog>(inf, inv, pf, pv);
    va[2 * b + 1] = wide_bits<Wide>(inv);
    __threadfence();
    st[2 * b + 1] = tag | (inf << 1) | 1ull;
    s_pv = pv;
    s_pf = pf;
  }
  __syncthreads();
  if (t == 0 || t >= a.n_tiles || !f) return;
  Wide c = ev;
  uint32_t cf = ef;
  seg_combine<Prog>(cf, c, s_pf, s_pv);
  const Wide totalw = Prog::wcombine(c, Prog::widen(a.head_partial[t]));
  uint32_t vtx = i0;
  if (a.close_vtx) {
    vtx = a.close_vtx[i0];
    if (vtx == 0xFFFFFFFFu) return;
  }
  store_vertex<Prog>(a, vtx, Prog::narrow(totalw));
}

}
```

lux_b200/csrc/runtime.cuh:

```cuda
#pragma once
#include <vector>
#include "comm.h"
#include "common.cuh"
#include "panel.cuh"
#include "seg.cuh"
#include "push.cuh"
#include "bc.cuh"
#include "tc.cuh"
#include "kcore.cuh"
#include "truss.cuh"

struct FixupScratch {
  void* d_head = nullptr;
  void* d_tail = nullptr;
  void* d_carry = nullptr;
  uint32_t* d_carry_flag = nullptr;
  void* d_block_agg = nullptr;
  uint32_t* d_block_flag = nullptr;
  uint32_t n_fix_blocks = 0;
  unsigned long long* d_chain = nullptr;
  uint32_t chain_epoch = 0;
};

struct PullLayout {
  uint64_t* d_row_end = nullptr;
  uint32_t* d_row_end32 = nullptr;
  void* d_src = nullptr;
  uint32_t* d_tile_v = nullptr;
  uint32_t n_vtx = 0;
  uint64_t e_cnt = 0;
  uint32_t n_tiles = 0;
  FixupScratch fix;
  uint32_t* d_close = nullptr;
  uint32_t* d_empty = nullptr;
  uint32_t n_empty = 0;
  uint32_t* d_empty_hub = nullptr;
  uint32_t n_empty_hub = 0;
  uint32_t n_stages = 0;
  uint64_t n_words = 0;
};

struct SweepSettings {
  bool seg = true;
  int main_shape = 6, panel_shape = 1, cs_shape = 6;
  int sb = -1;
  uint32_t sb_bs = 0;
  uint32_t sb_blocks = 48;
  uint32_t sb_min_indeg = 64;
  int sb_tier = -1;
  double sb_slot_edges = 0.5;
  int cs = -1;
  double cs_seg_mb = 24.0;
  double hot_mb = 24.0;
  bool l2_persist = true;
  double l2_window_mb = -1.0;
};

struct PhaseTimer {
  bool on = false, per_call = false;
  std::vector<cudaEvent_t> ev;
  std::vector<int> tag;
  double sum[12] = {0};
  long cnt = 0;
};

struct CfState {
  uint32_t* chunk_first = nullptr;
  uint32_t* chunk_vtx = nullptr;
  uint32_t n_chunks = 0;
  float* partial = nullptr;
};

struct BcState {
  double* sigma = nullptr;
  double* delta = nullptr;
  double* scores = nullptr;
  uint32_t* order = nullptr;
  double* lvl = nullptr;
  uint64_t lvl_cap = 0;
  uint32_t* off = nullptr;
  uint64_t off_cap = 0;
  uint32_t* split = nullptr;
  uint64_t split_cap = 0;
  void* sort_tmp = nullptr;
  size_t sort_bytes = 0;
  uint32_t* ctl = nullptr;
  luxb::BcHub* hubs = nullptr;
  double* partial = nullptr;
  std::vector<uint32_t> h_off, h_split;
  bool has_source = false;
};

struct TcState {
  uint64_t m = 0;
  uint64_t* off = nullptr;
  uint32_t* dst = nullptr;
  uint32_t* staged = nullptr;
  uint64_t* stage_pre = nullptr;
  uint32_t* group = nullptr;
  uint32_t* big = nullptr;
  uint32_t n_group = 0, n_big = 0;
  unsigned long long* t = nullptr;
  unsigned long long* total = nullptr;
  unsigned int* next = nullptr;
  void* sum_tmp = nullptr;
  size_t sum_bytes = 0;
  int group_grid = 0, big_grid = 0;
};

struct KcoreState {
  uint64_t m = 0;
  uint64_t* off = nullptr;
  uint32_t* adj = nullptr;
  uint32_t* deg0 = nullptr;
  uint32_t* deg = nullptr;
  uint32_t* core = nullptr;
  uint32_t* alive[2] = {nullptr, nullptr};
  uint32_t* piece[2] = {nullptr, nullptr};
  uint32_t* f = nullptr;
  uint64_t* pre = nullptr;
  luxb::KcoreRec* rec = nullptr;
  luxb::KcoreRec* h_rec = nullptr;
  unsigned long long* bad = nullptr;
  void* scan_tmp = nullptr;
  size_t scan_bytes = 0;
  int grid = 0;
};

struct TrussState {
  uint64_t m = 0;
  uint32_t e_lo = 0, e_hi = 0;
  uint64_t* ekey = nullptr;
  TcState o;
  uint32_t* oid = nullptr;
  uint64_t* off = nullptr;
  uint64_t* adj = nullptr;
  uint32_t* sup0 = nullptr;
  uint32_t* sup = nullptr;
  uint32_t* truss = nullptr;
  uint8_t* st = nullptr;
  uint32_t* tv = nullptr;
  uint32_t* alive[2] = {nullptr, nullptr};
  uint32_t* piece[2] = {nullptr, nullptr};
  uint32_t* f = nullptr;
  uint64_t* pre = nullptr;
  luxb::KcoreRec* rec = nullptr;
  luxb::KcoreRec* h_rec = nullptr;
  unsigned long long* bad = nullptr;
  void* scan_tmp = nullptr;
  size_t scan_bytes = 0;
  int grid = 0;
  int group_grid = 0, big_grid = 0;
};

enum class MemKind : uint8_t { kDevice, kPinned, kMapped };
struct OwnedBuf { void* p; MemKind kind; };

struct luxb_graph {
  luxb_config cfg{};
  uint32_t nv = 0;
  uint64_t ne = 0;
  int P = 1;
  int parts_found = 0;
  bool weighted = false;

  uint32_t ref_rl[LUXB_MAX_PARTS]{};
  uint32_t ref_np[LUXB_MAX_PARTS]{};
  uint64_t ref_cl[LUXB_MAX_PARTS]{};
  uint32_t rl[LUXB_MAX_PARTS]{};
  uint32_t np[LUXB_MAX_PARTS]{};
  uint64_t cl[LUXB_MAX_PARTS]{};
  uint32_t cap[LUXB_MAX_PARTS]{};
  uint64_t slot_off[LUXB_MAX_PARTS]{};
  uint64_t slot_bytes[LUXB_MAX_PARTS]{};
  uint64_t fq_total = 0;

  uint32_t row_left = 0, n_part = 0;
  uint64_t col_left = 0, e_part = 0;
  uint64_t* d_row_end = nullptr;
  uint32_t* d_src = nullptr;
  int32_t* d_weight = nullptr;
  PullLayout base;
  int pull_shape = 0;

  cudaStream_t stream = nullptr;
  cudaEvent_t ev_begin = nullptr, ev_end = nullptr;
  int num_sms = 0;

  bool inited = false;
  uint32_t* d_deg = nullptr;
  void* d_val[2] = {nullptr, nullptr};
  int cur = 0;
  uint32_t hot_n = 0;
  void* d_hot = nullptr;
  uint32_t hot_off[LUXB_MAX_PARTS + 1]{};
  uint32_t* d_hot_order = nullptr;
  uint32_t* d_src_gather = nullptr;
  bool packed = false;
  uint32_t cold_n = 0;
  uint32_t cold_off[LUXB_MAX_PARTS + 1]{};
  uint32_t* d_zperm = nullptr;
  uint32_t* d_pack_list = nullptr;
  float* d_xt[2] = {nullptr, nullptr};
  int cur_xt = 0;
  uint64_t xt_hot_chunk = 0, xt_cold_chunk = 0;
  cudaStream_t stream2 = nullptr;
  cudaEvent_t ev_pack = nullptr, ev_cold = nullptr;
  bool cold_pending = false;

  void* peer_xt[2][LUXB_MAX_PARTS]{};
  bool replica_stale = false;
  uint32_t* d_cur = nullptr;
  uint64_t* d_out_end = nullptr;
  uint32_t* d_out_dst = nullptr;
  int32_t* d_out_w = nullptr;
  void* d_big_list = nullptr;
  uint32_t big_capacity = 0;
  unsigned char* d_fq_all = nullptr;
  unsigned char* d_fq_new = nullptr;
  unsigned char* d_fq_tmp = nullptr;
  uint32_t* d_hdr_all = nullptr;
  luxb::FrontierCtl* d_fctl = nullptr;
  uint64_t* d_slot_off = nullptr;
  uint32_t* h_hdr = nullptr;
  uint32_t* h_scratch = nullptr;
  unsigned long long* d_counters = nullptr;
  CfState cf;
  BcState bc;
  TcState tc;
  KcoreState kc;
  TrussState tr;

  luxb::ncclComm_t comm = nullptr;
  bool p2p_ready = false;
  void* peer_val[2][LUXB_MAX_PARTS]{};
  void* peer_fq[LUXB_MAX_PARTS]{};
  uint32_t* d_sync = nullptr;
  uint32_t* d_flags = nullptr;
  void* peer_flags[LUXB_MAX_PARTS]{};
  uint32_t barrier_epoch = 0;
  uint32_t* h_barrier_err = nullptr;
  uint64_t barrier_timeout_ns = 30000000000ull;
  bool flag_barrier = true;
  bool flag_barrier_all = false;
  bool direct_push = false;

  SweepSettings sweep;

  bool empties_done[2] = {false, false};
  bool seg_on = false;
  bool sb_on = false;
  PullLayout sb_main, sb_panel;
  uint32_t sb_n_hub = 0, sb_n_blocks = 0, sb_n_groups = 0, sb_bs = 0;
  uint32_t* d_hub_vtx = nullptr;
  uint32_t* d_hub_bits = nullptr;
  uint32_t* d_sb_partial = nullptr;
  luxb::SplitGroups sb_groups{};
  uint32_t sb_super_end[luxb::kPanelMaxBlocks]{};
  bool cold_z = false;
  bool cs_on = false;
  PullLayout sb_cold;

  int pull_ctas = 3;
  bool overlap_exchange = true;
  bool fused_fixup = true;
  int panel_reserve_sms = 12;
  int l2_hints = 1;
  PhaseTimer pt;

  bool kernel_timing = false;
  std::vector<cudaEvent_t> kt_events;
  size_t kt_used = 0;

  std::vector<OwnedBuf> owned;

  luxb_stats_t stats{};
  std::vector<uint64_t> trace_active;
  std::vector<int32_t> trace_pull;
};
```

lux_b200/csrc/seg.cuh:

```cuda
#pragma once
#include "common.cuh"
#include "programs.cuh"
#include "pull.cuh"
#include "panel.cuh"

namespace luxb {

constexpr uint32_t kDummyVtx = 0xFFFFFFFFu;

template <int kWarps_, int kStages_, int kRounds_, bool kPanel_, int kTab_, int kV_ = 8>
struct SegShape {
  static constexpr int kWarps = kWarps_;
  static constexpr int kThreads = 32 * (kWarps + 1);
  static constexpr int kStages = kStages_;
  static constexpr int kRounds = kRounds_;
  static constexpr bool kPanel = kPanel_;
  static constexpr int kTab = kTab_;
  static constexpr int kV = kV_;
  static constexpr int kRound = 32 * kV;
  static constexpr int kPiece = kRounds * kRound;
  static constexpr int kStageEdges = kWarps * kPiece;
  static constexpr int kWordBytes = kPanel ? 2 : 4;
  static constexpr int kStageBytes = kStageEdges * kWordBytes;
  static constexpr int kSumElems = kRound + 8;
  static constexpr int kHdrElems = kWarps + 4;
  static constexpr size_t kSmemBytes = (size_t)kTab * 4 + (size_t)kStages * kStageBytes + (size_t)kWarps * kSumElems * 4 +
                                       (2 * kStages + 1) * 8 + (size_t)kStages * kHdrElems * 4 + 16;
  static_assert(!kPanel || (kTab > 0 && kTab <= 32768 && kTab % 4 == 0), "panel offsets are 15 bit");
  static_assert(kStageBytes % 16 == 0, "TMA bulk copies move multiples of 16 bytes");
  static_assert(kV == 8 || kV == 16, "a lane reads its words with 128-bit loads");
};

template <class Prog>
struct SegArgs {
  PullArgs<Prog> p;
  const void* words;
  uint32_t n_stages;
  uint32_t* tile_counter;
  uint32_t bs, n_blocks;
  uint32_t super_end[kPanelMaxBlocks];
};

template <class Prog, class Shape>
__global__ void __launch_bounds__(Shape::kThreads, Shape::kPanel ? 1 : 2) seg_tile_kernel(const __grid_constant__ SegArgs<Prog> a) {
  using Acc = typename Prog::Acc;
  using Vertex = typename Prog::Vertex;
  using Wide = typename Prog::Wide;
  constexpr int kStages = Shape::kStages, kWarps = Shape::kWarps, kRounds = Shape::kRounds, kV = Shape::kV;
  constexpr bool kPanel = Shape::kPanel;
  static_assert(sizeof(Acc) == 4 && sizeof(Vertex) == 4, "4-byte vertex values");

  extern __shared__ __align__(128) unsigned char smem_raw[];
  Vertex* tab = reinterpret_cast<Vertex*>(smem_raw);
  unsigned char* w_buf = smem_raw + (size_t)Shape::kTab * 4;
  Acc* sums_all = reinterpret_cast<Acc*>(w_buf + (size_t)kStages * Shape::kStageBytes);
  uint64_t* full = reinterpret_cast<uint64_t*>(sums_all + (size_t)kWarps * Shape::kSumElems);
  uint64_t* empty = full + kStages;
  uint64_t* tab_full = empty + kStages;
  uint32_t* hdr_all = reinterpret_cast<uint32_t*>(tab_full + 1);

  const int lane = threadIdx.x & 31, warp = threadIdx.x >> 5;

  if (threadIdx.x == 0) {
    for (int s = 0; s < kStages; ++s) { mbar_init(&full[s], 1); mbar_init(&empty[s], kWarps); }
    mbar_init(tab_full, 1);
    fence_mbar_init();
  }
  __syncthreads();

  if (warp == kWarps) {
    const uint64_t policy = l2_policy_evict_first();
    uint32_t cur_b = 0, gen = 0;
    bool loaded = false;
    for (uint32_t n = 0;; ++n) {
      const int s = n % kStages;
      if (n >= (uint32_t)kStages) mbar_wait(&empty[s], ((n / kStages) - 1) & 1u);
      uint32_t T = 0;
      if (lane == 0) T = atomicAdd(a.tile_counter, 1u);
      T = __shfl_sync(0xffffffffu, T, 0);
      uint32_t* hdr = hdr_all + s * Shape::kHdrElems;
      if (T >= a.n_stages) {
        if (lane == 0) { hdr[0] = 0xFFFFFFFFu; mbar_arrive(&full[s]); }
        break;
      }
      if (kPanel) {
        uint32_t b = cur_b;
        while (b + 1 < a.n_blocks && T >= a.super_end[b]) ++b;
        if (!loaded || b != cur_b) {
          for (int q = 0; q < kStages; ++q) {
            if (n > (uint32_t)q) {
              const uint32_t m = n - 1 - ((n - 1 - q) % kStages);
              mbar_wait(&empty[q], (m / kStages) & 1u);
            }
          }
          cur_b = b;
          loaded = true;
          ++gen;
          if (lane == 0) {
            const uint32_t bytes = a.bs * 4u;
            mbar_arrive_expect_tx(tab_full, bytes);
            const char* gsrc = reinterpret_cast<const char*>(a.p.x_hot + (size_t)b * a.bs);
            char* sdst = reinterpret_cast<char*>(tab);
            const uint64_t keep = l2_policy_evict_last();
            for (uint32_t off = 0; off < bytes; off += 32768u) {
              const uint32_t chunk = bytes - off < 32768u ? bytes - off : 32768u;
              bulk_g2s(sdst + off, gsrc + off, chunk, tab_full, keep);
            }
          }
          __syncwarp();
        }
      }
      const uint64_t t0 = (uint64_t)T * kWarps;
      if (lane <= kWarps) hdr[2 + lane] = __ldg(a.p.tile_v + t0 + lane);
      __syncwarp();
      if (lane == 0) {
        hdr[0] = T;
        hdr[1] = gen;
        mbar_arrive_expect_tx(&full[s], (uint32_t)Shape::kStageBytes);
        const char* gsrc = reinterpret_cast<const char*>(a.words) + (size_t)T * Shape::kStageBytes;
        char* sdst = reinterpret_cast<char*>(w_buf) + (size_t)s * Shape::kStageBytes;
        for (uint32_t off = 0; off < (uint32_t)Shape::kStageBytes; off += 32768u) {
          const uint32_t chunk = Shape::kStageBytes - off < 32768u ? Shape::kStageBytes - off : 32768u;
          bulk_g2s(sdst + off, gsrc + off, chunk, &full[s], policy);
        }
      }
      __syncwarp();
    }
    return;
  }

  Acc* sums = sums_all + (size_t)warp * Shape::kSumElems;
  uint32_t my_gen = 0;
  const uint64_t pol_hot = a.p.l2_hints ? l2_policy_evict_last() : l2_policy_evict_normal();
  const uint64_t pol_cold = a.p.l2_hints ? l2_policy_evict_first() : l2_policy_evict_normal();
  for (uint32_t n = 0;; ++n) {
    const int s = n % kStages;
    mbar_wait(&full[s], (n / kStages) & 1u);
    const uint32_t* hdr = hdr_all + s * Shape::kHdrElems;
    const uint32_t T = hdr[0];
    if (T == 0xFFFFFFFFu) break;
    if (kPanel) {
      const uint32_t gen = hdr[1];
      if (gen != my_gen) { mbar_wait(tab_full, (gen - 1) & 1u); my_gen = gen; }
    }
    const uint32_t t = T * kWarps + warp;
    const uint32_t jbase = hdr[2 + warp];
    const unsigned char* P = w_buf + (size_t)s * Shape::kStageBytes + (size_t)warp * Shape::kPiece * Shape::kWordBytes;

    Wide carry = Prog::widen(Prog::identity());
    bool seen = false;
    uint32_t n_closed = 0;

#pragma unroll 1
    for (int r = 0; r < kRounds; ++r) {
      uint32_t id[kV];
      uint32_t fm = 0;
      if (kPanel) {
        const uint4* src = reinterpret_cast<const uint4*>(P + ((size_t)r * Shape::kRound + lane * kV) * 2);
#pragma unroll
        for (int c = 0; c < kV / 8; ++c) {
          const uint4 q = src[c];
          const uint32_t w4[4] = {q.x, q.y, q.z, q.w};
#pragma unroll
          for (int k = 0; k < 4; ++k) {
            id[8 * c + 2 * k] = w4[k] & 0x7FFFu;
            id[8 * c + 2 * k + 1] = (w4[k] >> 16) & 0x7FFFu;
            fm |= ((w4[k] >> 15) & 1u) << (8 * c + 2 * k);
            fm |= (w4[k] >> 31) << (8 * c + 2 * k + 1);
          }
        }
      } else {
        const uint4* src = reinterpret_cast<const uint4*>(P + ((size_t)r * Shape::kRound + lane * kV) * 4);
#pragma unroll
        for (int c = 0; c < kV / 4; ++c) {
          const uint4 q = src[c];
          const uint32_t w4[4] = {q.x, q.y, q.z, q.w};
#pragma unroll
          for (int k = 0; k < 4; ++k) {
            id[4 * c + k] = w4[k] & 0x7FFFFFFFu;
            fm |= (w4[k] >> 31) << (4 * c + k);
          }
        }
      }
      Acc val[kV];
#pragma unroll
      for (int k = 0; k < kV; ++k) {
        if (kPanel) {
          val[k] = Prog::gather(tab[id[k]]);
        } else {
          const bool hot = id[k] < a.p.hot_n;
          const Vertex* ptr = hot ? a.p.x_hot + id[k] : a.p.x_old + (id[k] - a.p.hot_n);
          val[k] = Prog::gather(gather_load_l2(ptr, hot, pol_hot, pol_cold));
        }
      }
      if (r == kRounds - 1) {
        __syncwarp();
        if (lane == 0) mbar_arrive(&empty[s]);
      }
      const uint32_t cnt = __popc(fm);
      uint32_t incl = cnt;
#pragma unroll
      for (int off = 1; off < 32; off <<= 1) {
        const uint32_t up = __shfl_up_sync(0xffffffffu, incl, off);
        if (lane >= off) incl += up;
      }
      const uint32_t excl = incl - cnt;
      const uint32_t n_round = __shfl_sync(0xffffffffu, incl, 31);
      constexpr int kPre = kV / 4;
      uint32_t vpre[kPre];
#pragma unroll
      for (int q = 0; q < kPre; ++q) {
        const uint32_t li = lane + 32 * q;
        vpre[q] = li < n_round ? __ldg(a.p.close_vtx + jbase + n_closed + li) : kDummyVtx;
      }
      Acc run = Prog::identity(), first_val = Prog::identity();
      uint32_t h = 0;
      if (kPanel) {
#pragma unroll
        for (int k = 0; k < kV; ++k) {
          const bool f = (fm >> k) & 1u;
          const Acc closed = run;
          if (f && h != 0) sums[excl + h] = closed;
          first_val = (f && h == 0) ? closed : first_val;
          run = f ? val[k] : Prog::combine(run, val[k]);
          h += f ? 1u : 0u;
        }
      } else {
#pragma unroll
        for (int k = 0; k < kV; ++k) {
          if ((fm >> k) & 1u) {
            if (h == 0) first_val = run; else sums[excl + h] = run;
            run = Prog::identity();
            ++h;
          }
          run = Prog::combine(run, val[k]);
        }
      }
      Acc sv = run;
      uint32_t sf = cnt ? 1u : 0u;
#pragma unroll
      for (int off = 1; off < 32; off <<= 1) {
        const Acc pv = __shfl_up_sync(0xffffffffu, sv, off);
        const uint32_t pf = __shfl_up_sync(0xffffffffu, sf, off);
        if (lane >= off) {
          if (!sf) sv = Prog::combine(pv, sv);
          sf |= pf;
        }
      }
      Acc ex_v = __shfl_up_sync(0xffffffffu, sv, 1);
      if (lane == 0) ex_v = Prog::identity();
      const Acc tail31 = __shfl_sync(0xffffffffu, sv, 31);
      const unsigned heads = __ballot_sync(0xffffffffu, cnt != 0);
      const bool defer_first = !seen;
      if (cnt) {
        const Acc value = Prog::combine(ex_v, first_val);
        if (lane == __ffs(heads) - 1) {
          const Wide tot = Prog::wcombine(carry, Prog::widen(value));
          if (defer_first) a.p.head_partial[t] = Prog::narrow(tot); else sums[0] = Prog::narrow(tot);
        } else {
          sums[excl] = value;
        }
      }
      if (heads) { carry = Prog::widen(tail31); seen = true; } else { carry = Prog::wcombine(carry, Prog::widen(tail31)); }
      __syncwarp();
      auto finish = [&](uint32_t li, uint32_t v) {
        if (li == 0 && defer_first) return;
        if (v == kDummyVtx) return;
        if (kPanel) a.p.out[v] = sums[li];
        else store_vertex<Prog>(a.p, v, sums[li]);
      };
#pragma unroll
      for (int q = 0; q < kPre; ++q) {
        const uint32_t li = lane + 32 * q;
        if (li < n_round) finish(li, vpre[q]);
      }
      for (uint32_t li = lane + 32 * kPre; li < n_round; li += 32) finish(li, __ldg(a.p.close_vtx + jbase + n_closed + li));
      n_closed += n_round;
      __syncwarp();
    }
    if (lane == 0) a.p.tail_partial[t] = Prog::narrow(carry);
  }
}

struct StreamBlocks {
  uint32_t n_blocks;
  uint32_t vfirst[kPanelMaxBlocks + 1];
  uint64_t ebase[kPanelMaxBlocks + 1];
  uint64_t wbase[kPanelMaxBlocks + 1];
  uint64_t hshift[kPanelMaxBlocks + 1];
};

template <class T>
__device__ __forceinline__ uint32_t find_block(const T* first, uint32_t n, uint64_t x) {
  uint32_t lo = 0, hi = n;
  while (hi - lo > 1) {
    const uint32_t mid = (lo + hi) >> 1;
    if ((uint64_t)first[mid] <= x) lo = mid; else hi = mid;
  }
  return lo;
}

__global__ void nonempty_flag_kernel(const uint64_t* __restrict__ row_end, uint32_t n_vtx, uint32_t* __restrict__ flag) {
  for (uint64_t i = (uint64_t)blockIdx.x * blockDim.x + threadIdx.x; i < n_vtx; i += (uint64_t)gridDim.x * blockDim.x)
    flag[i] = row_end[i] > (i == 0 ? 0 : row_end[i - 1]) ? 1u : 0u;
}

template <class Word>
__global__ void stream_heads_kernel(const uint64_t* __restrict__ row_end, uint32_t n_vtx, const uint32_t* __restrict__ flag,
                                    const uint32_t* __restrict__ segrank, const __grid_constant__ StreamBlocks sb,
                                    Word* __restrict__ words, uint32_t* __restrict__ close_list, uint32_t vtx_offset) {
  constexpr Word kHead = (Word)1 << (sizeof(Word) * 8 - 1);
  for (uint64_t i = (uint64_t)blockIdx.x * blockDim.x + threadIdx.x; i < n_vtx; i += (uint64_t)gridDim.x * blockDim.x) {
    if (!flag[i]) continue;
    const uint32_t b = find_block(sb.vfirst, sb.n_blocks, i);
    const uint64_t begin = i == 0 ? 0 : row_end[i - 1];
    words[begin - sb.ebase[b] + sb.wbase[b]] |= kHead;
    close_list[1 + (uint64_t)segrank[i] + sb.hshift[b]] = (uint32_t)i + vtx_offset;
  }
}

template <class Word, class In>
__global__ void stream_copy_kernel(const In* __restrict__ ids, uint64_t e_cnt, const __grid_constant__ StreamBlocks sb,
                                   Word* __restrict__ words) {
  for (uint64_t e = (uint64_t)blockIdx.x * blockDim.x + threadIdx.x; e < e_cnt; e += (uint64_t)gridDim.x * blockDim.x) {
    const uint32_t b = find_block(sb.ebase, sb.n_blocks, e);
    words[e - sb.ebase[b] + sb.wbase[b]] = (Word)ids[e];
  }
}

template <class Word>
__global__ void stream_pad_kernel(Word* __restrict__ words, uint64_t from, uint64_t to) {
  constexpr Word kHead = (Word)1 << (sizeof(Word) * 8 - 1);
  for (uint64_t e = from + (uint64_t)blockIdx.x * blockDim.x + threadIdx.x; e < to; e += (uint64_t)gridDim.x * blockDim.x) words[e] = kHead;
}

template <class Word>
__global__ void piece_heads_kernel(const Word* __restrict__ words, uint32_t n_pieces, uint32_t piece, uint32_t* __restrict__ cnt) {
  constexpr Word kHead = (Word)1 << (sizeof(Word) * 8 - 1);
  const unsigned lane = threadIdx.x & 31;
  const uint64_t warps_total = ((uint64_t)gridDim.x * blockDim.x) >> 5;
  for (uint64_t t = ((uint64_t)blockIdx.x * blockDim.x + threadIdx.x) >> 5; t < n_pieces; t += warps_total) {
    uint32_t c = 0;
    for (uint32_t k = lane; k < piece; k += 32) c += (words[t * piece + k] & kHead) ? 1u : 0u;
#pragma unroll
    for (int off = 16; off; off >>= 1) c += __shfl_xor_sync(0xffffffffu, c, off);
    if (lane == 0) cnt[t] = c;
  }
}

__global__ void empty_split_kernel(const uint32_t* __restrict__ flag, uint32_t n_vtx, const uint32_t* __restrict__ hub_bits,
                                   uint32_t* __restrict__ plain, uint32_t* __restrict__ hubs, unsigned int* __restrict__ cursors) {
  const unsigned lane = threadIdx.x & 31;
  const uint64_t n_round = ((uint64_t)n_vtx + 31) & ~31ull;
  for (uint64_t i = (uint64_t)blockIdx.x * blockDim.x + threadIdx.x; i < n_round; i += (uint64_t)gridDim.x * blockDim.x) {
    const bool e = i < n_vtx && !flag[i];
    const bool hub = e && hub_bits != nullptr && ((hub_bits[i >> 5] >> (i & 31)) & 1u);
    const unsigned mp = __ballot_sync(0xffffffffu, e && !hub), mh = __ballot_sync(0xffffffffu, hub);
    unsigned bp = 0, bh = 0;
    if (lane == 0) {
      if (mp) bp = atomicAdd(cursors + 0, (unsigned)__popc(mp));
      if (mh) bh = atomicAdd(cursors + 1, (unsigned)__popc(mh));
    }
    bp = __shfl_sync(0xffffffffu, bp, 0);
    bh = __shfl_sync(0xffffffffu, bh, 0);
    if (e && !hub) plain[bp + __popc(mp & ((1u << lane) - 1))] = (uint32_t)i;
    if (hub) hubs[bh + __popc(mh & ((1u << lane) - 1))] = (uint32_t)i;
  }
}

template <class Prog>
__global__ void empties_kernel(const __grid_constant__ PullArgs<Prog> a, const uint32_t* __restrict__ empty_vtx, uint32_t n_empty) {
  for (uint64_t k = (uint64_t)blockIdx.x * blockDim.x + threadIdx.x; k < n_empty; k += (uint64_t)gridDim.x * blockDim.x)
    store_vertex<Prog>(a, empty_vtx[k], Prog::identity());
}

}
```

Measured before the change: 173,400.

## Store panel partials compactly by slot rank using presence bitmaps

Panel and cold-hub segment streams now write partial sums to a dense slot index computed per piece (piece_slot) instead of looking up a close-vertex list per segment. Only (group, hub) pairs that actually have edges get a slot. A bitmap with prefix popcounts lets the combine kernel locate each partial. This removes the close_vtx loads in the segment kernel, removes the full memset of the partial buffer, and shrinks the partial array. In exchange the combine step does extra bitmap/prefix loads and popc work, and the cold-hub path is now restricted to PageRank.

After: 187,500 (median of 6 runs). +8.2%, better.

```diff
diff --git a/lux_b200/csrc/api.cu b/lux_b200/csrc/api.cu
--- a/lux_b200/csrc/api.cu
+++ b/lux_b200/csrc/api.cu
@@ -3,6 +3,7 @@
 #include <stdlib.h>
 #include <string.h>
 #include <algorithm>
+#include <type_traits>
 #include <new>
 
 #include "build.cuh"
@@ -1264,7 +1265,7 @@
 }
 
 template <class Prog>
-static int launch_fixup(luxb_graph* g, const PullArgs<Prog>& a, FixupScratch& f) {
+static int launch_fixup(luxb_graph* g, const PullArgs<Prog>& a, FixupScratch& f, const uint2* piece_slot = nullptr) {
   if (a.n_tiles <= 1) return 0;
   if (g->fused_fixup) {
     if (!f.d_chain) {
@@ -1282,14 +1283,14 @@
       LUXB_CUDA(cudaMemsetAsync(f.d_chain, 0, (4ull * f.n_fix_blocks + 4) * 8, g->stream));
       f.chain_epoch = ch.epoch = 1;
     }
-    pull_fixup_fused_kernel<Prog><<<f.n_fix_blocks, kFixBlock, 0, g->stream>>>(a, ch);
+    pull_fixup_fused_kernel<Prog><<<f.n_fix_blocks, kFixBlock, 0, g->stream>>>(a, ch, piece_slot);
     LUXB_CUDA(cudaGetLastError());
     g->stats.kernel_launches++;
     return 0;
   }
   pull_fixup_scan_kernel<Prog><<<f.n_fix_blocks, kFixBlock, 0, g->stream>>>(a);
   pull_fixup_blocks_kernel<Prog><<<1, 1024, 0, g->stream>>>(a, f.n_fix_blocks);
-  pull_fixup_apply_kernel<Prog><<<f.n_fix_blocks, kFixBlock, 0, g->stream>>>(a);
+  pull_fixup_apply_kernel<Prog><<<f.n_fix_blocks, kFixBlock, 0, g->stream>>>(a, piece_slot);
   LUXB_CUDA(cudaGetLastError());
   g->stats.kernel_launches += 3;
   return 0;
@@ -1387,8 +1388,8 @@
 extern "C++" {
 template <class Word, class In>
 static int build_seg_stream(luxb_graph* g, PullLayout& L, const uint64_t* d_row_end, uint32_t n_vtx, const In* d_ids, uint64_t e_cnt,
-                            StreamBlocks& blk, uint32_t stage_edges, uint32_t piece, uint32_t vtx_offset, bool want_empty,
-                            const uint32_t* hub_bits, uint32_t* super_end) {
+                            StreamBlocks& blk, uint32_t stage_edges, uint32_t piece, bool want_empty, const uint32_t* hub_bits,
+                            uint32_t* super_end, bool slots = false, uint32_t slot_base = 0) {
   const int grid = g->num_sms * 8;
   DevTmp tmp;
   L = PullLayout();
@@ -1432,9 +1433,11 @@
   LUXB_CUDA(cudaGetLastError());
   const uint64_t n_heads = (uint64_t)n_seg + pads_total;
   LUXB_ARG(n_heads < 0xFFFFFFF0ull, "too many segments");
-  LUXB_TRY(gmalloc(g, &L.d_close, n_heads + 2));
-  LUXB_CUDA(cudaMemsetAsync(L.d_close, 0xFF, (n_heads + 2) * 4, g->stream));
-  stream_heads_kernel<Word><<<grid, 256, 0, g->stream>>>(d_row_end, n_vtx, d_flag, d_rank, blk, d_words, L.d_close, vtx_offset);
+  if (!slots) {
+    LUXB_TRY(gmalloc(g, &L.d_close, n_heads + 2));
+    LUXB_CUDA(cudaMemsetAsync(L.d_close, 0xFF, (n_heads + 2) * 4, g->stream));
+  }
+  stream_heads_kernel<Word><<<grid, 256, 0, g->stream>>>(d_row_end, n_vtx, d_flag, d_rank, blk, d_words, L.d_close);
   LUXB_CUDA(cudaGetLastError());
   uint32_t* d_cnt = nullptr;
   LUXB_TRY(tmp.alloc(&d_cnt, (uint64_t)L.n_tiles + 2));
@@ -1447,6 +1450,13 @@
   }));
   uint32_t heads_counted = 0;
   LUXB_CUDA(cudaMemcpyAsync(&heads_counted, L.d_tile_v + L.n_tiles, 4, cudaMemcpyDeviceToHost, g->stream));
+  if (slots) {
+    LUXB_ARG((uint64_t)slot_base + n_seg < 0x7FFFFFF0ull, "too many slots");
+    LUXB_TRY(gmalloc(g, &L.d_piece_slot, (uint64_t)L.n_tiles + 1));
+    piece_slot_kernel<<<grid_for(L.n_tiles, 256, grid), 256, 0, g->stream>>>(L.d_tile_v, L.n_tiles, piece, d_rank, blk, slot_base, L.d_piece_slot);
+    LUXB_CUDA(cudaGetLastError());
+    L.n_slots = n_seg;
+  }
   unsigned int* d_cur2 = nullptr;
   if (want_empty) {
     const uint32_t n_e = n_vtx - n_seg;
@@ -1478,13 +1488,14 @@
   blk.vfirst[1] = g->n_part;
   blk.ebase[1] = e_cnt;
   return build_seg_stream<uint32_t, uint32_t>(g, g->sb_main, d_row_end, g->n_part, d_ids, e_cnt, blk, (uint32_t)shp.stage_edges,
-                                              (uint32_t)shp.piece, 0, true, hub_bits, nullptr);
+                                              (uint32_t)shp.piece, true, hub_bits, nullptr);
 }
 
 extern "C++" {
 template <class Word>
 static int build_group_stream(luxb_graph* g, PullLayout& L, const uint16_t* d_key, const uint64_t* d_pay, uint64_t e_cnt, uint32_t g0,
-                              uint32_t g1, const unsigned long long* hist, uint32_t bs, const SegShapeInfo& shp, uint32_t* super_end) {
+                              uint32_t g1, const unsigned long long* hist, uint32_t bs, const SegShapeInfo& shp, uint32_t* super_end,
+                              uint32_t* d_bits, uint32_t slot_base) {
   const int grid = g->num_sms * 8;
   const uint32_t* vbase = g->sb_groups.vbase;
   const uint32_t v0 = vbase[g0], n_vtx = vbase[g1] - v0;
@@ -1502,6 +1513,8 @@
   LUXB_TRY(cub_call(tmp, g->stream, [&](void* t, size_t& b) {
     return cub::DeviceScan::InclusiveSum(t, b, d_vrow, d_vrow, (int)n_vtx, g->stream);
   }));
+  slot_bits_kernel<<<grid, 256, 0, g->stream>>>(d_vcount, g->sb_groups, g0, g1, v0, d_bits);
+  LUXB_CUDA(cudaGetLastError());
   tmp.release(d_vcount);
   StreamBlocks blk{};
   blk.n_blocks = super_end ? g1 - g0 : 1;
@@ -1509,8 +1522,8 @@
     blk.vfirst[b + 1] = super_end ? vbase[g0 + b + 1] - v0 : n_vtx;
     blk.ebase[b + 1] = super_end ? blk.ebase[b] + hist[g0 + b] : e_cnt;
   }
-  return build_seg_stream<Word, Word>(g, L, d_vrow, n_vtx, d_ids, e_cnt, blk, (uint32_t)shp.stage_edges, (uint32_t)shp.piece, v0, false,
-                                      nullptr, super_end);
+  return build_seg_stream<Word, Word>(g, L, d_vrow, n_vtx, d_ids, e_cnt, blk, (uint32_t)shp.stage_edges, (uint32_t)shp.piece, false,
+                                      nullptr, super_end, true, slot_base);
 }
 }
 
@@ -1662,17 +1675,38 @@
 
   const uint32_t NG = NB + S;
   LUXB_ARG(NG < kSplitKeyMain, "panel: too many source groups");
-  uint64_t n_slots = 0;
+  uint64_t n_pairs = 0, n_words = 0;
   g->sb_groups = SplitGroups{};
   for (uint32_t k = 0; k < NG; ++k) {
-    n_slots += k < NB ? n_pref[k] : Nh;
-    LUXB_ARG(n_slots < 0x7FFFFFF0ull, "panel: too many (group, hub) slots");
-    g->sb_groups.vbase[k + 1] = (uint32_t)n_slots;
-  }
-  LUXB_TRY(build_group_stream<uint16_t>(g, g->sb_panel, d_key2, d_pay2, e_cov, 0, NB, hist, bs, shp, g->sb_super_end));
+    const uint32_t n_k = k < NB ? n_pref[k] : Nh;
+    n_pairs += n_k;
+    n_words += (n_k + 31) / 32;
+    LUXB_ARG(n_pairs < 0x7FFFFFF0ull, "panel: too many (group, hub) pairs");
+    g->sb_groups.vbase[k + 1] = (uint32_t)n_pairs;
+    g->sb_groups.wbase[k + 1] = (uint32_t)n_words;
+  }
+  uint32_t *d_slot_bits = nullptr, *d_slot_pre = nullptr;
+  LUXB_TRY(tmp.alloc(&d_slot_bits, n_words + 1));
+  LUXB_TRY(tmp.alloc(&d_slot_pre, n_words + 1));
+  LUXB_TRY(build_group_stream<uint16_t>(g, g->sb_panel, d_key2, d_pay2, e_cov, 0, NB, hist, bs, shp, g->sb_super_end, d_slot_bits, 0));
   if (S)
     LUXB_TRY(build_group_stream<uint32_t>(g, g->sb_cold, d_key2 + e_cov, d_pay2 + e_cov, e_cold, NB, NG, hist, 0,
-                                          kSegMainInfo[st.cs_shape], nullptr));
+                                          kSegMainInfo[st.cs_shape], nullptr, d_slot_bits, g->sb_panel.n_slots));
+  const uint64_t n_slots = (uint64_t)g->sb_panel.n_slots + (S ? g->sb_cold.n_slots : 0);
+  popc_kernel<<<grid, 256, 0, g->stream>>>(d_slot_bits, n_words, d_slot_pre);
+  LUXB_CUDA(cudaMemsetAsync(d_slot_pre + n_words, 0, 4, g->stream));
+  LUXB_CUDA(cudaGetLastError());
+  LUXB_TRY(cub_call(tmp, g->stream, [&](void* t, size_t& b) {
+    return cub::DeviceScan::ExclusiveSum(t, b, d_slot_pre, d_slot_pre, (int)n_words + 1, g->stream);
+  }));
+  uint32_t kind_slots[4] = {0, 0, 0, 0};
+  const uint32_t kind_word[4] = {0, g->sb_groups.wbase[NB0], g->sb_groups.wbase[NB], (uint32_t)n_words};
+  for (int i = 0; i < 4; ++i) LUXB_CUDA(cudaMemcpyAsync(&kind_slots[i], d_slot_pre + kind_word[i], 4, cudaMemcpyDeviceToHost, g->stream));
+  LUXB_CUDA(cudaStreamSynchronize(g->stream));
+  if ((uint64_t)kind_slots[3] != n_slots) {
+    set_error("panel split: %u slots in the bitmap, %llu in the streams", kind_slots[3], (unsigned long long)n_slots);
+    return LUXB_ERR_STATE;
+  }
 
   uint32_t* d_main_src = nullptr;
   uint64_t* d_main_row = nullptr;
@@ -1695,10 +1729,10 @@
   tmp.release(d_main_src);
 
   LUXB_TRY(gmalloc(g, &g->d_sb_partial, (uint64_t)n_slots + 1));
-  LUXB_CUDA(cudaMemsetAsync(g->d_sb_partial, g->cfg.app == LUXB_SSSP || g->cfg.app == LUXB_BC ? 0xFF : 0, ((size_t)n_slots + 1) * 4, g->stream));
-  LUXB_CUDA(cudaStreamSynchronize(g->stream));
   g->d_hub_vtx = d_hub_vtx; tmp.keep(g, d_hub_vtx);
   g->d_hub_bits = d_hub_bits; tmp.keep(g, d_hub_bits);
+  g->d_slot_bits = d_slot_bits; tmp.keep(g, d_slot_bits);
+  g->d_slot_pre = d_slot_pre; tmp.keep(g, d_slot_pre);
   g->sb_n_hub = Nh;
   g->sb_n_blocks = NB;
   g->sb_n_groups = NG;
@@ -1714,11 +1748,15 @@
   g->stats.tier_blocks = NB - NB0;
   g->stats.tier_slots = NV - (uint64_t)NB0 * Nh;
   g->stats.tier_edges = e_cov - e_cov0;
-  if (g->cfg.verbose)
+  if (g->cfg.verbose) {
     printf("[luxb rank %d] source-blocked sweep: %u hub destinations (in-degree >= %u) x %u blocks of %u hot sources, + %u tier blocks "
            "(%llu slots, %llu edges); panel %llu edges (%.1f %%), cold-hub %llu edges (%u segments of %u values), main %llu edges\n",
            g->cfg.rank, Nh, st.sb_min_indeg, NB0, bs, NB - NB0, (unsigned long long)(NV - (uint64_t)NB0 * Nh), (unsigned long long)(e_cov - e_cov0),
            (unsigned long long)e_cov, 100.0 * e_cov / g->e_part, (unsigned long long)e_cold, S, cs.seg, (unsigned long long)e_main);
+    printf("[luxb rank %d] (group, hub) pairs with edges / all: tier 0 %u / %llu, tiers %u / %llu, cold segments %u / %llu\n", g->cfg.rank,
+           kind_slots[1], (unsigned long long)NB0 * Nh, kind_slots[2] - kind_slots[1], (unsigned long long)(NV - (uint64_t)NB0 * Nh),
+           kind_slots[3] - kind_slots[2], (unsigned long long)Nh * S);
+  }
   return 0;
 }
 
@@ -1747,19 +1785,20 @@
   return 0;
 }
 
-template <bool kPanel, class Prog>
+template <bool kPanel, class Prog, bool kSlots = kPanel>
 static int launch_seg_stream(luxb_graph* g, PullLayout& L, SegArgs<Prog>& a, int shape, int ctas_per_sm, int counter_slot, int tag,
                              const char* name) {
   a.p.tile_v = L.d_tile_v;
   a.p.n_tiles = L.n_tiles;
   fill_fixup_args(a.p, L.fix);
   a.p.close_vtx = L.d_close;
+  a.piece_slot = L.d_piece_slot;
   a.words = L.d_src;
   a.n_stages = L.n_stages;
   a.tile_counter = reinterpret_cast<uint32_t*>(g->d_counters + counter_slot);
   LUXB_CUDA(cudaMemsetAsync(a.tile_counter, 0, 4, g->stream));
 #define LUXB_CASE_MSHAPE(id, warps, stages, rounds) \
-  case id: LUXB_TRY((launch_seg_shape<Prog, SegMain##id>(g, a, ctas_per_sm))); break;
+  case id: LUXB_TRY((launch_seg_shape<Prog, std::conditional_t<kSlots, SlotShape<SegMain##id>, SegMain##id>>(g, a, ctas_per_sm))); break;
 #define LUXB_CASE_PSHAPE(id, warps, stages, rounds, tab, v) \
   case id: LUXB_TRY((launch_seg_shape<Prog, SegPanel##id>(g, a, ctas_per_sm))); break;
   if constexpr (kPanel) {
@@ -1775,7 +1814,7 @@
   }
   g->stats.kernel_launches++;
   pt_mark(g, tag);
-  return launch_fixup(g, a.p, L.fix);
+  return launch_fixup(g, a.p, L.fix, L.d_piece_slot);
 }
 }
 
@@ -1828,16 +1867,21 @@
     pt_mark(g, 1);
   }
   if (g->cs_on) {
-    SegArgs<Prog> ca{};
-    ca.p.x_old = x_cold;
-    ca.p.x_hot = reinterpret_cast<const typename Prog::Vertex*>(g->d_hot);
-    ca.p.hot_n = g->hot_n;
-    ca.p.out = reinterpret_cast<typename Prog::Vertex*>(g->d_sb_partial);
-    ca.p.raw_out = 1;
-    ca.p.l2_hints = 0;
-    ca.p.prm = prm;
-    LUXB_TRY((launch_seg_stream<false, Prog>(g, g->sb_cold, ca, g->sweep.cs_shape, g->pull_ctas, 4, 9, "cold-hub")));
-    pt_mark(g, 1);
+    if constexpr (std::is_same<Prog, PageRankProgram>::value) {
+      SegArgs<Prog> ca{};
+      ca.p.x_old = x_cold;
+      ca.p.x_hot = reinterpret_cast<const typename Prog::Vertex*>(g->d_hot);
+      ca.p.hot_n = g->hot_n;
+      ca.p.out = reinterpret_cast<typename Prog::Vertex*>(g->d_sb_partial);
+      ca.p.raw_out = 1;
+      ca.p.l2_hints = 0;
+      ca.p.prm = prm;
+      LUXB_TRY((launch_seg_stream<false, Prog, true>(g, g->sb_cold, ca, g->sweep.cs_shape, g->pull_ctas, 4, 9, "cold-hub")));
+      pt_mark(g, 1);
+    } else {
+      set_error("the cold-hub stream is built for PageRank only");
+      return LUXB_ERR_STATE;
+    }
   }
   LUXB_TRY((launch_seg_main<Prog>(g, g->sb_main, x_nat, x_cold, out_local, out_buffer, prm, g->sb_on ? g->d_hub_bits : nullptr)));
   LUXB_TRY(kt_end(g));
@@ -1849,6 +1893,8 @@
     ca.n_groups = g->sb_n_groups;
     ca.row_left = g->row_left;
     ca.sg = g->sb_groups;
+    ca.slot_bits = g->d_slot_bits;
+    ca.slot_pre = g->d_slot_pre;
     ca.partial = reinterpret_cast<const Acc*>(g->d_sb_partial);
     ca.x_nat = x_nat;
     ca.out = out_local;
diff --git a/lux_b200/csrc/panel.cuh b/lux_b200/csrc/panel.cuh
--- a/lux_b200/csrc/panel.cuh
+++ b/lux_b200/csrc/panel.cuh
@@ -11,6 +11,7 @@
 
 struct SplitGroups {
   uint32_t vbase[kSplitKeyMain + 1];
+  uint32_t wbase[kSplitKeyMain + 1];
 };
 
 __global__ void hub_flag_kernel(const uint64_t* __restrict__ row_end_rel, uint32_t n_part, uint32_t min_indeg,
@@ -133,11 +134,34 @@
   }
 }
 
+__global__ void slot_bits_kernel(const uint32_t* __restrict__ vcount, const __grid_constant__ SplitGroups sg, uint32_t g0, uint32_t g1,
+                                 uint32_t v0, uint32_t* __restrict__ bits) {
+  const unsigned lane = threadIdx.x & 31;
+  const uint64_t warps_total = ((uint64_t)gridDim.x * blockDim.x) >> 5;
+  for (uint64_t w = sg.wbase[g0] + (((uint64_t)blockIdx.x * blockDim.x + threadIdx.x) >> 5); w < sg.wbase[g1]; w += warps_total) {
+    uint32_t lo = g0, hi = g1;
+    while (hi - lo > 1) {
+      const uint32_t mid = (lo + hi) >> 1;
+      if (sg.wbase[mid] <= w) lo = mid; else hi = mid;
+    }
+    const uint32_t h = (uint32_t)(w - sg.wbase[lo]) * 32u + lane;
+    const bool f = h < sg.vbase[lo + 1] - sg.vbase[lo] && vcount[sg.vbase[lo] - v0 + h] != 0;
+    const unsigned m = __ballot_sync(0xffffffffu, f);
+    if (lane == 0) bits[w] = m;
+  }
+}
+
+__global__ void popc_kernel(const uint32_t* __restrict__ bits, uint64_t n, uint32_t* __restrict__ out) {
+  for (uint64_t i = (uint64_t)blockIdx.x * blockDim.x + threadIdx.x; i < n; i += (uint64_t)gridDim.x * blockDim.x) out[i] = __popc(bits[i]);
+}
+
 template <class Prog>
 struct CombineArgs {
   const uint32_t* hub_vtx;
   uint32_t n_hub, n_blocks, n_groups, row_left;
   SplitGroups sg;
+  const uint32_t* slot_bits;
+  const uint32_t* slot_pre;
   const typename Prog::Acc* partial;
   const typename Prog::Vertex* x_nat;
   typename Prog::Vertex* out;
@@ -151,17 +175,31 @@
     typename Prog::Acc raw0;
     memcpy(&raw0, &a.out[v], sizeof(raw0));
     typename Prog::Wide t = Prog::widen(raw0);
+    const uint32_t w = (uint32_t)(h >> 5), me = 1u << (h & 31), below = me - 1u;
+    auto add8 = [&](uint32_t g) {
+      uint32_t bits[8], pre[8];
+#pragma unroll
+      for (int i = 0; i < 8; ++i) {
+        bits[i] = __ldg(a.slot_bits + a.sg.wbase[g + i] + w);
+        pre[i] = __ldg(a.slot_pre + a.sg.wbase[g + i] + w);
+      }
+      typename Prog::Acc p[8];
+#pragma unroll
+      for (int i = 0; i < 8; ++i) p[i] = (bits[i] & me) ? a.partial[pre[i] + __popc(bits[i] & below)] : Prog::identity();
+#pragma unroll
+      for (int i = 0; i < 8; ++i)
+        if (bits[i] & me) t = Prog::wcombine(t, Prog::widen(p[i]));
+    };
+    auto add = [&](uint32_t g) {
+      const uint32_t bits = __ldg(a.slot_bits + a.sg.wbase[g] + w);
+      if (bits & me) t = Prog::wcombine(t, Prog::widen(a.partial[__ldg(a.slot_pre + a.sg.wbase[g] + w) + __popc(bits & below)]));
+    };
     uint32_t b = 0;
-    for (; b + 8 <= a.n_blocks && h < a.sg.vbase[b + 8] - a.sg.vbase[b + 7]; b += 8) {
-      typename Prog::Acc p[8];
-#pragma unroll
-      for (int i = 0; i < 8; ++i) p[i] = a.partial[a.sg.vbase[b + i] + h];
-#pragma unroll
-      for (int i = 0; i < 8; ++i) t = Prog::wcombine(t, Prog::widen(p[i]));
-    }
-    for (; b < a.n_blocks && h < a.sg.vbase[b + 1] - a.sg.vbase[b]; ++b)
-      t = Prog::wcombine(t, Prog::widen(a.partial[a.sg.vbase[b] + h]));
-    for (uint32_t k = a.n_blocks; k < a.n_groups; ++k) t = Prog::wcombine(t, Prog::widen(a.partial[a.sg.vbase[k] + h]));
+    for (; b + 8 <= a.n_blocks && h < a.sg.vbase[b + 8] - a.sg.vbase[b + 7]; b += 8) add8(b);
+    for (; b < a.n_blocks && h < a.sg.vbase[b + 1] - a.sg.vbase[b]; ++b) add(b);
+    uint32_t k = a.n_blocks;
+    for (; k + 8 <= a.n_groups; k += 8) add8(k);
+    for (; k < a.n_groups; ++k) add(k);
     const typename Prog::Vertex oldv = Prog::kNeedsOld ? a.x_nat[a.row_left + v] : typename Prog::Vertex();
     const typename Prog::Vertex nv_ = Prog::update(a.row_left + v, Prog::narrow(t), oldv, a.prm);
     a.out[v] = nv_;
diff --git a/lux_b200/csrc/pull.cuh b/lux_b200/csrc/pull.cuh
--- a/lux_b200/csrc/pull.cuh
+++ b/lux_b200/csrc/pull.cuh
@@ -63,6 +63,9 @@
   const uint32_t* close_vtx;
 };
 
+constexpr uint32_t kSlotLo = 0x80000000u;
+__device__ __forceinline__ bool piece_slot_real(uint2 ps, uint32_t k) { return k >= (ps.y >> 31) && k < (ps.y & ~kSlotLo); }
+
 template <class Prog>
 __device__ __forceinline__ bool store_raw(const PullArgs<Prog>& a, uint32_t v) {
   if (a.raw_out) return true;
@@ -418,7 +421,7 @@
 }
 
 template <class Prog>
-__global__ void __launch_bounds__(kFixBlock) pull_fixup_apply_kernel(const __grid_constant__ PullArgs<Prog> a) {
+__global__ void __launch_bounds__(kFixBlock) pull_fixup_apply_kernel(const __grid_constant__ PullArgs<Prog> a, const uint2* __restrict__ piece_slot) {
   using Wide = typename Prog::Wide;
   const uint32_t t = blockIdx.x * kFixBlock + threadIdx.x;
   if (t == 0 || t >= a.n_tiles) return;
@@ -428,7 +431,11 @@
   if (!a.carry_flag[t]) c = Prog::wcombine(a.block_agg[blockIdx.x], c);
   Wide totalw = Prog::wcombine(c, Prog::widen(a.head_partial[t]));
   uint32_t v = i0;
-  if (a.close_vtx) {
+  if (piece_slot) {
+    const uint2 ps = piece_slot[t];
+    if (!piece_slot_real(ps, 0)) return;
+    v = ps.x;
+  } else if (a.close_vtx) {
     v = a.close_vtx[i0];
     if (v == 0xFFFFFFFFu) return;
   }
@@ -457,7 +464,8 @@
 }
 
 template <class Prog>
-__global__ void __launch_bounds__(kFixBlock) pull_fixup_fused_kernel(const __grid_constant__ PullArgs<Prog> a, const FixupChain<Prog> ch) {
+__global__ void __launch_bounds__(kFixBlock) pull_fixup_fused_kernel(const __grid_constant__ PullArgs<Prog> a, const FixupChain<Prog> ch,
+                                                                  const uint2* __restrict__ piece_slot) {
   using Wide = typename Prog::Wide;
   __shared__ Wide s_v[kFixBlock / 32];
   __shared__ uint32_t s_f[kFixBlock / 32];
@@ -543,7 +551,11 @@
   seg_combine<Prog>(cf, c, s_pf, s_pv);
   const Wide totalw = Prog::wcombine(c, Prog::widen(a.head_partial[t]));
   uint32_t vtx = i0;
-  if (a.close_vtx) {
+  if (piece_slot) {
+    const uint2 ps = piece_slot[t];
+    if (!piece_slot_real(ps, 0)) return;
+    vtx = ps.x;
+  } else if (a.close_vtx) {
     vtx = a.close_vtx[i0];
     if (vtx == 0xFFFFFFFFu) return;
   }
diff --git a/lux_b200/csrc/runtime.cuh b/lux_b200/csrc/runtime.cuh
--- a/lux_b200/csrc/runtime.cuh
+++ b/lux_b200/csrc/runtime.cuh
@@ -32,6 +32,8 @@
   uint32_t n_tiles = 0;
   FixupScratch fix;
   uint32_t* d_close = nullptr;
+  uint2* d_piece_slot = nullptr;
+  uint32_t n_slots = 0;
   uint32_t* d_empty = nullptr;
   uint32_t n_empty = 0;
   uint32_t* d_empty_hub = nullptr;
@@ -255,6 +257,8 @@
   uint32_t* d_hub_vtx = nullptr;
   uint32_t* d_hub_bits = nullptr;
   uint32_t* d_sb_partial = nullptr;
+  uint32_t* d_slot_bits = nullptr;
+  uint32_t* d_slot_pre = nullptr;
   luxb::SplitGroups sb_groups{};
   uint32_t sb_super_end[luxb::kPanelMaxBlocks]{};
   bool cold_z = false;
diff --git a/lux_b200/csrc/seg.cuh b/lux_b200/csrc/seg.cuh
--- a/lux_b200/csrc/seg.cuh
+++ b/lux_b200/csrc/seg.cuh
@@ -15,6 +15,7 @@
   static constexpr int kStages = kStages_;
   static constexpr int kRounds = kRounds_;
   static constexpr bool kPanel = kPanel_;
+  static constexpr bool kSlots = kPanel_;
   static constexpr int kTab = kTab_;
   static constexpr int kV = kV_;
   static constexpr int kRound = 32 * kV;
@@ -31,6 +32,11 @@
   static_assert(kV == 8 || kV == 16, "a lane reads its words with 128-bit loads");
 };
 
+template <class Base>
+struct SlotShape : Base {
+  static constexpr bool kSlots = true;
+};
+
 template <class Prog>
 struct SegArgs {
   PullArgs<Prog> p;
@@ -39,6 +45,7 @@
   uint32_t* tile_counter;
   uint32_t bs, n_blocks;
   uint32_t super_end[kPanelMaxBlocks];
+  const uint2* piece_slot;
 };
 
 template <class Prog, class Shape>
@@ -47,7 +54,7 @@
   using Vertex = typename Prog::Vertex;
   using Wide = typename Prog::Wide;
   constexpr int kStages = Shape::kStages, kWarps = Shape::kWarps, kRounds = Shape::kRounds, kV = Shape::kV;
-  constexpr bool kPanel = Shape::kPanel;
+  constexpr bool kPanel = Shape::kPanel, kSlots = Shape::kSlots;
   static_assert(sizeof(Acc) == 4 && sizeof(Vertex) == 4, "4-byte vertex values");
 
   extern __shared__ __align__(128) unsigned char smem_raw[];
@@ -146,6 +153,12 @@
     const uint32_t t = T * kWarps + warp;
     const uint32_t jbase = hdr[2 + warp];
     const unsigned char* P = w_buf + (size_t)s * Shape::kStageBytes + (size_t)warp * Shape::kPiece * Shape::kWordBytes;
+    uint32_t slot0 = 0, slot_end = 0;
+    if constexpr (kSlots) {
+      const uint2 ps = __ldg(a.piece_slot + t);
+      slot0 = ps.x;
+      slot_end = ps.y & ~kSlotLo;
+    }
 
     Wide carry = Prog::widen(Prog::identity());
     bool seen = false;
@@ -206,12 +219,14 @@
       }
       const uint32_t excl = incl - cnt;
       const uint32_t n_round = __shfl_sync(0xffffffffu, incl, 31);
-      constexpr int kPre = kV / 4;
+      constexpr int kPre = kSlots ? 1 : kV / 4;
       uint32_t vpre[kPre];
-#pragma unroll
-      for (int q = 0; q < kPre; ++q) {
-        const uint32_t li = lane + 32 * q;
-        vpre[q] = li < n_round ? __ldg(a.p.close_vtx + jbase + n_closed + li) : kDummyVtx;
+      if constexpr (!kSlots) {
+#pragma unroll
+        for (int q = 0; q < kPre; ++q) {
+          const uint32_t li = lane + 32 * q;
+          vpre[q] = li < n_round ? __ldg(a.p.close_vtx + jbase + n_closed + li) : kDummyVtx;
+        }
       }
       Acc run = Prog::identity(), first_val = Prog::identity();
       uint32_t h = 0;
@@ -269,12 +284,22 @@
         if (kPanel) a.p.out[v] = sums[li];
         else store_vertex<Prog>(a.p, v, sums[li]);
       };
-#pragma unroll
-      for (int q = 0; q < kPre; ++q) {
-        const uint32_t li = lane + 32 * q;
-        if (li < n_round) finish(li, vpre[q]);
-      }
-      for (uint32_t li = lane + 32 * kPre; li < n_round; li += 32) finish(li, __ldg(a.p.close_vtx + jbase + n_closed + li));
+      if constexpr (kSlots) {
+        for (uint32_t li = lane; li < n_round; li += 32) {
+          const uint32_t k = n_closed + li;
+          if (li == 0 && defer_first) continue;
+          if (k >= slot_end) break;
+          if (kPanel) a.p.out[slot0 + k] = sums[li];
+          else store_vertex<Prog>(a.p, slot0 + k, sums[li]);
+        }
+      } else {
+#pragma unroll
+        for (int q = 0; q < kPre; ++q) {
+          const uint32_t li = lane + 32 * q;
+          if (li < n_round) finish(li, vpre[q]);
+        }
+        for (uint32_t li = lane + 32 * kPre; li < n_round; li += 32) finish(li, __ldg(a.p.close_vtx + jbase + n_closed + li));
+      }
       n_closed += n_round;
       __syncwarp();
     }
@@ -308,14 +333,14 @@
 template <class Word>
 __global__ void stream_heads_kernel(const uint64_t* __restrict__ row_end, uint32_t n_vtx, const uint32_t* __restrict__ flag,
                                     const uint32_t* __restrict__ segrank, const __grid_constant__ StreamBlocks sb,
-                                    Word* __restrict__ words, uint32_t* __restrict__ close_list, uint32_t vtx_offset) {
+                                    Word* __restrict__ words, uint32_t* __restrict__ close_list) {
   constexpr Word kHead = (Word)1 << (sizeof(Word) * 8 - 1);
   for (uint64_t i = (uint64_t)blockIdx.x * blockDim.x + threadIdx.x; i < n_vtx; i += (uint64_t)gridDim.x * blockDim.x) {
     if (!flag[i]) continue;
     const uint32_t b = find_block(sb.vfirst, sb.n_blocks, i);
     const uint64_t begin = i == 0 ? 0 : row_end[i - 1];
     words[begin - sb.ebase[b] + sb.wbase[b]] |= kHead;
-    close_list[1 + (uint64_t)segrank[i] + sb.hshift[b]] = (uint32_t)i + vtx_offset;
+    if (close_list) close_list[1 + (uint64_t)segrank[i] + sb.hshift[b]] = (uint32_t)i;
   }
 }
 
@@ -345,6 +370,19 @@
 #pragma unroll
     for (int off = 16; off; off >>= 1) c += __shfl_xor_sync(0xffffffffu, c, off);
     if (lane == 0) cnt[t] = c;
+  }
+}
+
+__global__ void piece_slot_kernel(const uint32_t* __restrict__ tile_v, uint32_t n_pieces, uint32_t piece, const uint32_t* __restrict__ segrank,
+                                  const __grid_constant__ StreamBlocks sb, uint32_t slot_base, uint2* __restrict__ piece_slot) {
+  for (uint64_t t = (uint64_t)blockIdx.x * blockDim.x + threadIdx.x; t < n_pieces; t += (uint64_t)gridDim.x * blockDim.x) {
+    const uint32_t b = find_block(sb.wbase, sb.n_blocks, t * piece);
+    const int64_t r0 = segrank[sb.vfirst[b]], r1 = segrank[sb.vfirst[b + 1]];
+    const int64_t hb = r0 + (int64_t)sb.hshift[b];
+    const int64_t i0 = tile_v[t], i1 = tile_v[t + 1];
+    const int64_t last = i1 < hb + 1 + (r1 - r0) ? i1 : hb + 1 + (r1 - r0);
+    const int64_t end = last > i0 ? last - i0 : 0;
+    piece_slot[t] = make_uint2((uint32_t)((int64_t)slot_base + i0 - 1 - (int64_t)sb.hshift[b]), (uint32_t)end | (i0 == hb ? kSlotLo : 0u));
   }
 }
 
```
